# Kaixhin/Rainbow

Measured on AMD Instinct MI355X. Metric: gradient-steps/sec (batch=32, atoms=51), higher is better.
Workload: dtype f32; 1 GPU; pong-canonical-b32; architecture=canonical, batch_per_gpu=32, global_batch=32, atoms=51, actions=6, multi_step=3, replay_capacity_per_gpu=1000000, parallelism=single device

## Files before the change

rainbow_amd/csrc/adam_body.h:

```cpp
#pragma once
#include "rb_common.h"

struct ClipAdamArgs {
  float* p; float* g; float* m; float* v;
  int64_t n;
  const float* part; int nparts;
  float max_norm; float* norm_out;
  float w1, b2, w2, neg_step_size, bc2_sqrt, eps;
  const long long* step_dev;
  double lr, beta1, beta2;
  int64_t skip_lo4, skip_len4;
  const int32_t* batch_status;
  int64_t pair_mu4, pair_len4;
  unsigned hole_lo4, hole4;
  int pair_blk0;
  int pair_f4, pair_split_row;
  float tau;
  const float* pair_eout;
  const float* pair_ein;
  int32_t* pair_clipped;
  float* t;
};
static_assert(sizeof(ClipAdamArgs) <= 256, "ClipAdamArgs: the device copy (adam_args_dev, rb_debug_adam_pass) is 256 bytes");
__device__ __forceinline__ void rb_adam_elem(float& p, float& g, float& m, float& v, float coef, const ClipAdamArgs& a) {
  g = g * coef;
  m = fmaf(a.w1, g - m, m);
  v = v * a.b2 + a.w2 * g * g;
  const float denom = sqrtf(v) / a.bc2_sqrt + a.eps;
  p = p + a.neg_step_size * (m / denom);
}
__device__ __forceinline__ void rb_adam_quad(float4& P, float4& G, float4& M, float4& V, float coef, const ClipAdamArgs& a) {
  rb_adam_elem(P.x, G.x, M.x, V.x, coef, a);
  rb_adam_elem(P.y, G.y, M.y, V.y, coef, a);
  rb_adam_elem(P.z, G.z, M.z, V.z, coef, a);
  rb_adam_elem(P.w, G.w, M.w, V.w, coef, a);
}

__device__ __forceinline__ void rb_ema_elem(float& t, float p, float tau) {
  t = fmaf(tau, p - t, t);
}
__device__ __forceinline__ void rb_ema_quad(float4& T, const float4& P, float tau, bool copy) {
  if (copy) { T = P; return; }
  rb_ema_elem(T.x, P.x, tau); rb_ema_elem(T.y, P.y, tau); rb_ema_elem(T.z, P.z, tau); rb_ema_elem(T.w, P.w, tau);
}

struct rb_adam_req {
  float status;
  unsigned st_lo, st_hi;
  float pv[16];
};
__device__ __forceinline__ void rb_adam_hosted_request(const ClipAdamArgs& a, rb_adam_req& q) {
  const unsigned T = blockDim.x;
  q.status = 0.0f;
  if (a.batch_status) q.status = rb_ld1_buf(rb_make_buf(a.batch_status), 0, 0);
  const rb_buf bs = rb_make_buf(a.step_dev);
  q.st_lo = __builtin_bit_cast(unsigned, rb_ld1_buf(bs, 0, 0)); q.st_hi = __builtin_bit_cast(unsigned, rb_ld1_buf(bs, 4, 0));
  const rb_buf bpart = rb_make_buf(a.part);
#pragma unroll
  for (int u = 0; u < 16; ++u) {
    const int i = (int)threadIdx.x + u * (int)T;
    q.pv[u] = rb_ld1_buf(bpart, 4u * (unsigned)(i < a.nparts ? i : a.nparts - 1), 0);
  }
}
__device__ __forceinline__ bool rb_adam_hosted_prologue(ClipAdamArgs& a, int eb, const rb_adam_req& q, float* s_red16, float* coef_out) {
  const unsigned T = blockDim.x;
  float acc = 0.0f;
#pragma unroll
  for (int u = 0; u < 16; ++u)
    if ((int)threadIdx.x + u * (int)T < a.nparts) acc += q.pv[u];
  {
    const rb_buf bpart = rb_make_buf(a.part);
    for (int i0 = (int)threadIdx.x + 16 * (int)T; i0 < a.nparts; i0 += 16 * (int)T) {
      float pv[16];
#pragma unroll
      for (int u = 0; u < 16; ++u) {
        const int i = i0 + u * (int)T;
        pv[u] = rb_ld1_buf(bpart, 4u * (unsigned)(i < a.nparts ? i : a.nparts - 1), 0);
      }
#pragma unroll
      for (int u = 0; u < 16; ++u)
        if (i0 + u * (int)T < a.nparts) acc += pv[u];
    }
  }
  if (threadIdx.x == 0) {
    const double t = (double)(long long)(((unsigned long long)q.st_hi << 32) | q.st_lo);
    const double bc1 = 1.0 - pow(a.beta1, t), bc2 = 1.0 - pow(a.beta2, t);
    s_red16[16] = (float)(-(a.lr / bc1));
    s_red16[17] = (float)sqrt(bc2);
  }
  acc = rb_block_sum(acc, s_red16);
  if (rb_wave_uniform(__builtin_bit_cast(int, q.status)) != 0) {
    if (eb == 0 && threadIdx.x == 0 && a.norm_out) rb_st1_wt(a.norm_out, 0, 0.0f);
    return false;
  }
  const float total = sqrtf(acc);
  float coef = a.max_norm / (total + 1e-6f);
  if (coef > 1.0f) coef = 1.0f;
  if (eb == 0 && threadIdx.x == 0 && a.norm_out) rb_st1_wt(a.norm_out, 0, total);
  a.neg_step_size = s_red16[16];
  a.bc2_sqrt = s_red16[17];
  *coef_out = coef;
  return true;
}

template <bool EMA>
__device__ __forceinline__ void rb_adam_hosted_pairs(ClipAdamArgs& a, int eb, int pb, float* s_red16) {
  constexpr int PU = 2;
  const unsigned T = blockDim.x;
  const unsigned len4 = (unsigned)a.pair_len4, mu4 = (unsigned)a.pair_mu4;
  const unsigned base = (unsigned)pb * (T * PU) + threadIdx.x;
  rb_adam_req q;
  rb_adam_hosted_request(a, q);
  const rb_buf beo = rb_make_buf(a.pair_eout), bei = rb_make_buf(a.pair_ein);
  float4 E[PU];
  float eo[PU];
#pragma unroll
  for (int u = 0; u < PU; ++u) {
    unsigned j = base + u * T;
    if (j >= len4) j = len4 - 1;
    const unsigned row = j / (unsigned)a.pair_f4, cq = j - row * (unsigned)a.pair_f4;
    eo[u] = rb_ld1_buf(beo, 4 * row, 0);
    E[u] = rb_ld4_buf(bei, 16 * (cq + ((int)row >= a.pair_split_row ? (unsigned)a.pair_f4 : 0u)), 0);
  }
  const rb_buf bp = rb_make_buf(a.p), bg = rb_make_buf(a.g), bm = rb_make_buf(a.m), bv = rb_make_buf(a.v);
  float4 P[PU], G[PU], M[PU], V[PU], P2[PU], M2[PU], V2[PU];
#pragma unroll
  for (int u = 0; u < PU; ++u) {
    unsigned j = base + u * T;
    if (j >= len4) j = len4 - 1;
    const unsigned i = mu4 + j, i2 = i + len4;
    P[u] = rb_ld4_buf(bp, 16 * i, 0); G[u] = rb_ld4_buf(bg, 16 * i, 0);
    M[u] = rb_ld4_buf(bm, 16 * i, 0); V[u] = rb_ld4_buf(bv, 16 * i, 0);
    P2[u] = rb_ld4_buf(bp, 16 * i2, 0); M2[u] = rb_ld4_buf(bm, 16 * i2, 0); V2[u] = rb_ld4_buf(bv, 16 * i2, 0);
  }
  const bool ema_copy = EMA && a.tau == 1.0f;
  float4 TG[EMA ? PU : 1], TG2[EMA ? PU : 1];
  if (EMA && !ema_copy) {
    const rb_buf bt = rb_make_buf(a.t);
#pragma unroll
    for (int u = 0; u < PU; ++u) {
      unsigned j = base + u * T;
      if (j >= len4) j = len4 - 1;
      TG[u] = rb_ld4_buf(bt, 16 * (mu4 + j), 0); TG2[u] = rb_ld4_buf(bt, 16 * (mu4 + j + len4), 0);
    }
  }
  float coef;
  if (!rb_adam_hosted_prologue(a, eb, q, s_red16, &coef)) return;
  if (pb == 0 && threadIdx.x == 0 && a.pair_clipped) rb_st1_wt(reinterpret_cast<float*>(a.pair_clipped), 0, __builtin_bit_cast(float, coef < 1.0f ? 1 : 0));
#pragma unroll
  for (int u = 0; u < PU; ++u) {
    const unsigned j = base + u * T;
    if (j >= len4) continue;
    const unsigned i = mu4 + j, i2 = i + len4;
    float4 pr;
    pr.x = eo[u] * E[u].x; pr.y = eo[u] * E[u].y; pr.z = eo[u] * E[u].z; pr.w = eo[u] * E[u].w;
    float4 G2;
    G2.x = G[u].x * pr.x; G2.y = G[u].y * pr.y; G2.z = G[u].z * pr.z; G2.w = G[u].w * pr.w;
    rb_adam_quad(P[u], G[u], M[u], V[u], coef, a);
    rb_adam_quad(P2[u], G2, M2[u], V2[u], coef, a);
    rb_st4_wt(a.p, 16 * i, P[u]); rb_st4_wt(a.m, 16 * i, M[u]); rb_st4_wt(a.v, 16 * i, V[u]);
    rb_st4_wt(a.p, 16 * i2, P2[u]); rb_st4_wt(a.m, 16 * i2, M2[u]); rb_st4_wt(a.v, 16 * i2, V2[u]);
    if (coef < 1.0f) { rb_st4_wt(a.g, 16 * i, G[u]); rb_st4_wt(a.g, 16 * i2, G2); }
    if (EMA) {
      rb_ema_quad(TG[u], P[u], a.tau, ema_copy); rb_ema_quad(TG2[u], P2[u], a.tau, ema_copy);
      rb_st4_wt(a.t, 16 * i, TG[u]); rb_st4_wt(a.t, 16 * i2, TG2[u]);
    }
  }
}

template <int UNROLL, bool EMA = false>
__device__ __forceinline__ void rb_adam_hosted_block(const ClipAdamArgs* ad, int eb, int nblk, float* s_red16 ) {
  ClipAdamArgs a = rb_ld_uniform(ad);
  const int nplain = a.hole4 > 0 ? a.pair_blk0 : nblk;
  if (eb >= nplain) {
    rb_adam_hosted_pairs<EMA>(a, eb, eb - nplain, s_red16);
    return;
  }
  const unsigned T = blockDim.x;
  const unsigned n4 = (unsigned)(a.n >> 2);
  const unsigned hole_lo = a.hole4 > 0 ? a.hole_lo4 : n4, hole = a.hole4;
  const unsigned nv4 = n4 - hole;
  auto real_of = [&](unsigned j) { return j < hole_lo ? j : j + hole; };
  const unsigned base = (unsigned)eb * (T * UNROLL) + threadIdx.x;
  const rb_buf bp = rb_make_buf(a.p), bg = rb_make_buf(a.g), bm = rb_make_buf(a.m), bv = rb_make_buf(a.v);
  rb_adam_req q;
  rb_adam_hosted_request(a, q);
  float4 P[UNROLL], G[UNROLL], M[UNROLL], V[UNROLL];
#pragma unroll
  for (int u = 0; u < UNROLL; ++u) {
    unsigned j = base + u * T;
    if (j >= nv4) j = nv4 > 0 ? nv4 - 1 : 0;
    const unsigned i = real_of(j);
    P[u] = rb_ld4_buf(bp, 16 * i, 0); G[u] = rb_ld4_buf(bg, 16 * i, 0);
    M[u] = rb_ld4_buf(bm, 16 * i, 0); V[u] = rb_ld4_buf(bv, 16 * i, 0);
  }
  const bool ema_copy = EMA && a.tau == 1.0f;
  const bool has_tail = eb == nplain - 1 && ((a.n >> 2) << 2) + threadIdx.x < a.n;
  const unsigned tail_off = (unsigned)(4 * (((a.n >> 2) << 2) + threadIdx.x));
  float4 TG[EMA ? UNROLL : 1];
  float tg_tail = 0.0f;
  if (EMA && !ema_copy) {
    const rb_buf bt = rb_make_buf(a.t);
#pragma unroll
    for (int u = 0; u < UNROLL; ++u) {
      unsigned j = base + u * T;
      if (j >= nv4) j = nv4 > 0 ? nv4 - 1 : 0;
      TG[u] = rb_ld4_buf(bt, 16 * real_of(j), 0);
    }
    if (has_tail) tg_tail = rb_ld1_buf(bt, tail_off, 0);
  }
  float coef;
  if (!rb_adam_hosted_prologue(a, eb, q, s_red16, &coef)) return;
#pragma unroll
  for (int u = 0; u < UNROLL; ++u) {
    const unsigned j = base + u * T;
    if (j >= nv4) continue;
    const unsigned i = real_of(j);
    rb_adam_quad(P[u], G[u], M[u], V[u], coef, a);
    rb_st4_wt(a.p, 16 * i, P[u]); rb_st4_wt(a.m, 16 * i, M[u]); rb_st4_wt(a.v, 16 * i, V[u]);
    if (coef < 1.0f) rb_st4_wt(a.g, 16 * i, G[u]);
    if (EMA) {
      rb_ema_quad(TG[u], P[u], a.tau, ema_copy);
      rb_st4_wt(a.t, 16 * i, TG[u]);
    }
  }
  if (eb == nplain - 1) {
    const int64_t t = ((a.n >> 2) << 2) + threadIdx.x;
    if (t < a.n) {
      const unsigned o = (unsigned)(4 * t);
      float p = rb_ld1_buf(bp, o, 0), g = rb_ld1_buf(bg, o, 0), m = rb_ld1_buf(bm, o, 0), v = rb_ld1_buf(bv, o, 0);
      rb_adam_elem(p, g, m, v, coef, a);
      rb_st1_wt(a.p, o, p); rb_st1_wt(a.m, o, m); rb_st1_wt(a.v, o, v);
      if (coef < 1.0f) rb_st1_wt(a.g, o, g);
      if (EMA) {
        if (ema_copy) tg_tail = p; else rb_ema_elem(tg_tail, p, a.tau);
        rb_st1_wt(a.t, o, tg_tail);
      }
    }
  }
}

int rb_launch_adam_pending(const ClipAdamArgs* args_dev, int blocks, void* stream, bool ema = false);
```

rainbow_amd/csrc/conv_dispatch.h:

```cpp
#pragma once
#include "learner_plan.h"

static PlanIn plan_in(const rb_learner* l) {
  return PlanIn{l->L, l->opt, l->caps, l->n_cu, l->flags, l->world > 1 && l->fact_local != nullptr && l->caps.fast_fc, l->sink != nullptr};
}

template <class C>
static int launch_conv_fwd(rb_learner* l, int layer, int n_on, int n_tg, const ImgSrc& src, const NetPtrs& on,
                           const NetPtrs& tg, hipStream_t stream) {
  using G = typename C::G;
  constexpr int NT = C::NT, PR = C::PR, KMAX = C::KMAX, PCH = C::PCH;
  constexpr bool FIRST = C::FIRST;
  const ConvLayer& c = l->L.conv[layer];
  const ConvFwdPlan p = plan_conv_fwd_g<C>(plan_in(l), layer, n_on, n_tg, src.f32 != nullptr);
  if (p.kernel == CONV_FWD_GEMM) {
    if (layer == 0) {
      ConvFwdProb<G, true> q;
      q.cin = c.cin; q.cout = c.cout;
      q.n_img[0] = n_on; q.n_img[1] = n_tg; q.img_base[0] = 0; q.img_base[1] = n_on;
      q.w[0] = on.conv_w[0]; q.w[1] = tg.conv_w[0]; q.bias[0] = on.conv_b[0]; q.bias[1] = tg.conv_b[0];
      q.src = src; q.in_f = nullptr; q.out = l->act[0];
      RB_LAUNCH((k_gemm<1, 2, ConvFwdProb<G, true>>), p.grid, dim3(p.block), stream, q);
    } else {
      ConvFwdProb<G, false> q;
      q.cin = c.cin; q.cout = c.cout;
      q.n_img[0] = n_on; q.n_img[1] = n_tg; q.img_base[0] = 0; q.img_base[1] = n_on;
      q.w[0] = on.conv_w[layer]; q.w[1] = tg.conv_w[layer]; q.bias[0] = on.conv_b[layer]; q.bias[1] = tg.conv_b[layer];
      q.src = src; q.in_f = l->act[layer - 1]; q.out = l->act[layer];
      RB_LAUNCH((k_gemm<2, 1, ConvFwdProb<G, false>>), p.grid, dim3(p.block), stream, q);
    }
    RB_LAUNCH_CHECK();
    return RB_OK;
  }
  ConvLdsFwdArgs a;
  a.cin = c.cin; a.cout = c.cout; a.n_on = n_on;
  a.w[0] = on.conv_w[layer]; a.w[1] = tg.conv_w[layer]; a.bias[0] = on.conv_b[layer]; a.bias[1] = tg.conv_b[layer];
  a.src = src; a.in_f = layer > 0 ? l->act[layer - 1] : nullptr; a.out = l->act[layer];
  a.out_blocked = (layer == l->L.nconv - 1 && l->caps.fast_fc) ? l->feat_b : nullptr;
  a.rows_total = n_on + n_tg;
  a.ipb = p.ipb;
  a.img_fast = p.img_fast;
  static const char* const tags[3] = {"conv1_fwd:k_conv_fwd_lds", "conv2_fwd:k_conv_fwd_lds", "conv3_fwd:k_conv_fwd_lds"};
  const dim3 block(p.block);
  switch (p.kernel) {
    case CONV_FWD_FULL:
      if constexpr (FIRST && ConvFwdFullLds<G, KMAX>::FITS) { RB_LAUNCH_T(tags[layer], (k_conv_fwd_full<G, KMAX>), p.grid, block, stream, a); }
      break;
    case CONV_FWD_MULTI_T16:
      if constexpr (!FIRST && C::T16_OK) { RB_LAUNCH_T(tags[layer], (k_conv_fwd_multi_t16<G, NT, PR, KMAX, PCH>), p.grid, block, stream, a); }
      break;
    case CONV_FWD_T16:
      if constexpr (C::T16_OK) { RB_LAUNCH_T(tags[layer], (k_conv_fwd_t16<G, NT, PR, KMAX, FIRST, PCH, 1>), p.grid, block, stream, a); }
      break;
    case CONV_FWD_LDS_F32:
      if constexpr (FIRST) { RB_LAUNCH_T(tags[layer], (k_conv_fwd_lds<G, NT, PR, KMAX, FIRST, PCH, FIRST>), p.grid, block, stream, a); }
      break;
    case CONV_FWD_LDS:
      if constexpr (FIRST || !C::T16_OK) { RB_LAUNCH_T(tags[layer], (k_conv_fwd_lds<G, NT, PR, KMAX, FIRST, PCH>), p.grid, block, stream, a); }
      break;
    case CONV_FWD_GEMM: break;
  }
  RB_LAUNCH_CHECK();
  return RB_OK;
}

static int conv_fwd(rb_learner* l, int layer, int n_on, int n_tg, const ImgSrc& src, const NetPtrs& on,
                    const NetPtrs& tg, hipStream_t stream) {
  return with_geom(l->L.conv[layer], [&](auto cfg) { return launch_conv_fwd<decltype(cfg)>(l, layer, n_on, n_tg, src, on, tg, stream); });
}

template <class C>
static int launch_conv_dx(rb_learner* l, int layer, hipStream_t stream) {
  using G = typename C::G;
  const Layout& L = l->L;
  const ConvLayer& c = L.conv[layer];
  const ConvDxPlan p = plan_conv_dx_g<C>(plan_in(l), layer, l->lazy_dfeat != 0);
  if (p.kernel == CONV_DX_NONE) return RB_OK;
  if constexpr (G::IH != 84) {
    if (p.kernel == CONV_DX_GEMM) {
      ConvDxProb<G> q;
      q.B = L.B; q.cin = c.cin; q.cout = c.cout;
      q.w = l->p_online + L.conv_w[layer]; q.dy = l->dact[layer]; q.x_act = l->act[layer - 1]; q.dx = l->dact[layer - 1];
      if (c.cin <= 32) { RB_LAUNCH((k_gemm<1, 2, ConvDxProb<G>>), p.grid, dim3(p.block), stream, q); }
      else { RB_LAUNCH((k_gemm<2, 1, ConvDxProb<G>>), p.grid, dim3(p.block), stream, q); }
      RB_LAUNCH_CHECK();
      return RB_OK;
    }
    ConvLdsDxArgs a;
    a.cin = c.cin; a.cout = c.cout;
    a.w = l->p_online + L.conv_w[layer]; a.dy = l->dact[layer]; a.x_act = l->act[layer - 1]; a.dx = l->dact[layer - 1];
    a.wT = l->conv_wT[layer];
    constexpr bool lazy = RB_LAST_CONV_GEOM(G);
    a.dy_part = l->dfeat_part; a.dy_mask = l->act[layer]; a.dy_stride = (int64_t)L.B * L.F; a.dy_splits = lazy ? l->lazy_splits : 0;
    a.ipb = p.ipb; a.batch = L.B; a.img_fast = p.img_fast;
    constexpr int NT = ConvDxTiles<G>::NT;
    static const char* const tags[3] = {"conv1_dx:k_conv_dx_lds", "conv2_dx:k_conv_dx_lds", "conv3_dx:k_conv_dx_lds"};
    const dim3 block(p.block);
    switch (p.kernel) {
      case CONV_DX_T16_MULTI:
        if constexpr (dx_t16_geom(G::KS, G::S, G::IH)) { RB_LAUNCH_T(tags[layer], (k_conv_dx_t16_multi<G, 64, lazy>), p.grid, block, stream, a); }
        break;
      case CONV_DX_LDS_MULTI:
        if constexpr (!dx_t16_geom(G::KS, G::S, G::IH)) { RB_LAUNCH_T(tags[layer], (k_conv_dx_lds<G, NT, 64, lazy, true>), p.grid, block, stream, a); }
        break;
      case CONV_DX_LDS:
        RB_LAUNCH_T(tags[layer], (k_conv_dx_lds<G, NT, 64, lazy, false>), p.grid, block, stream, a);
        break;
      default: break;
    }
    RB_LAUNCH_CHECK();
  }
  return RB_OK;
}
static int conv_dx(rb_learner* l, int layer, hipStream_t stream) {
  return with_geom(l->L.conv[layer], [&](auto cfg) { return launch_conv_dx<decltype(cfg)>(l, layer, stream); });
}

template <class C>
static int launch_conv_dw_gemm(rb_learner* l, int layer, const uint8_t* states, hipStream_t stream) {
  using G = typename C::G;
  const Layout& L = l->L;
  const ConvLayer& c = L.conv[layer];
  const ConvDwGemmPlan p = plan_conv_dw_gemm(plan_in(l), layer);
  if (layer == 0) {
    ConvDwProb<G, true> q;
    q.B = L.B; q.cin = c.cin; q.cout = c.cout; q.splits = p.splits;
    q.dy = l->dact[0]; q.x_u8 = states; q.x_f = nullptr; q.part = l->dw_part[0];
    RB_LAUNCH((k_gemm<1, 2, ConvDwProb<G, true>>), p.grid, dim3(p.block), stream, q);
  } else {
    ConvDwProb<G, false> q;
    q.B = L.B; q.cin = c.cin; q.cout = c.cout; q.splits = p.splits;
    q.dy = l->dact[layer]; q.x_u8 = nullptr; q.x_f = l->act[layer - 1]; q.part = l->dw_part[layer];
    RB_LAUNCH((k_gemm<2, 2, ConvDwProb<G, false>>), p.grid, dim3(p.block), stream, q);
  }
  RB_LAUNCH_CHECK();
  l->dw_slices[layer] = p.splits;
  return RB_OK;
}
static int conv_dw_gemm(rb_learner* l, int layer, const uint8_t* states, hipStream_t stream) {
  return with_geom(l->L.conv[layer], [&](auto cfg) { return launch_conv_dw_gemm<decltype(cfg)>(l, layer, states, stream); });
}

static int conv_dw_all(rb_learner* l, hipStream_t stream) {
  const Layout& L = l->L;
  const ConvDwAllPlan p = plan_conv_dw_all(plan_in(l));
  ConvDwAllArgs a;
  a.batch = L.B;
  a.img_fast = p.img_fast;
  for (int i = 0; i < 3; ++i) { a.ipb[i] = p.ipb[i]; a.cotiles[i] = p.cotiles[i]; a.nblocks[i] = p.nblocks[i]; }
  for (int i = 0; i < L.nconv; ++i) {
    const ConvLayer& c = L.conv[i];
    ConvLdsDwArgs& d = a.layer[i];
    d.cin = c.cin; d.cout = c.cout; d.dy = l->dact[i]; d.part = l->dw_part[i];
    d.src = l->cur_src; d.x_f = i > 0 ? l->act[i - 1] : nullptr;
    d.dy_part = l->dfeat_part; d.dy_mask = l->act[i]; d.dy_stride = (int64_t)L.B * L.F;
    d.dy_splits = (l->lazy_dfeat && i == L.nconv - 1 && i > 0) ? l->lazy_splits : 0;
    l->dw_slices[i] = p.dw_slices[i];
  }
  for (int i = L.nconv; i < 3; ++i) a.layer[i] = a.layer[0];
  if (L.nconv == 3) {
    RB_LAUNCH_T("conv_dw_all", (k_conv_dw_all<GeomC1, 7, GeomC2, 9, 512, GeomC3, 7, 576, 3>), dim3(p.total), dim3(RB_CONV_THREADS), stream, a);
  } else {
    RB_LAUNCH_T("conv_dw_all", (k_conv_dw_all<GeomD1, 4, GeomD2, 3, 800, GeomD2, 3, 800, 2>), dim3(p.total), dim3(RB_CONV_THREADS), stream, a);
  }
  RB_LAUNCH_CHECK();
  return RB_OK;
}
```

rainbow_amd/csrc/conv_fwd.h:

```cpp
#pragma once
#include "conv_stage.h"
#include "kernel_stamp.h"

struct ConvLdsFwdArgs {
  int cin, cout;
  int n_on;
  const float* w[2];
  const float* bias[2];
  ImgSrc src;
  const float* in_f;
  float* out;
  float* out_blocked;
  int rows_total;
  int ipb;
  int img_fast;
};

template <class G>
__device__ __forceinline__ void rb_conv_store_out(const ConvLdsFwdArgs& a, int img, int m, int p, float o) {
  a.out[((int64_t)img * a.cout + m) * G::P + p] = o;
  if (a.out_blocked) a.out_blocked[rb_blocked_index(img, m * G::P + p, a.rows_total)] = o;
}

template <class G, int KMAX, int PLANE, int RP, int SUB>
__device__ __forceinline__ constexpr int rb_t16_off(int j) {
  return (j / G::KK) * PLANE + ((j % G::KK) / G::KS) * RP + (((j % G::KK) % G::KS) % G::S) * SUB + ((j % G::KK) % G::KS) / G::S;
}
template <class G, int NT, int PR, int KMAX, int T16 = 0>
struct ConvFwdLdsSize {
  static constexpr int KGRAN = 2 * RB_CONV_WAVES;
  static constexpr int KPAD = (KMAX + KGRAN - 1) / KGRAN * KGRAN;
  static constexpr int RED = RB_CONV_WAVES * 16 * 64;
  static constexpr int WS = KPAD + 4;
  static constexpr int CQ = (KMAX / G::KK) / 4;
  typedef ConvPatch<G, PR, T16 ? CQ : 0> PG;
  static constexpr int SUB = PG::SUB, RP = PG::RP, PLANE = PG::PLANE;
  static __device__ __forceinline__ constexpr int at(int j) { return rb_t16_off<G, KMAX, PLANE, RP, SUB>(j); }
  static constexpr int OPS = 32 * WS + (KMAX / G::KK) * PLANE;
  static constexpr int WSZ = T16 ? OPS : (OPS > RED ? OPS : RED);
  static constexpr int FLOATS = WSZ + (T16 ? 0 : KPAD);
};
template <class G, int NT, int PR, int KMAX, bool FIRST, int PCH = 32 * NT, bool F32SRC = false, int T16 = 0>
struct ConvFwdWaves {
  static constexpr int PT = (PCH + 15) / 16;
  static constexpr bool SPLIT_LAST = T16 == 1 && PT >= 3 && ((2 * PT) % 4) == 2 && ((KMAX / 4) % 8) == 0;
  static constexpr int TILE_WAVES = T16 == 1 ? (SPLIT_LAST ? 2 * PT + 2 : 2 * PT) : PT;
  static constexpr int PARTF = SPLIT_LAST ? 4 * 4 * 64 : 0;
  static constexpr int NWV = T16 == 0 ? RB_CONV_WAVES : (TILE_WAVES + 3) / 4 * 4;
};

struct ConvT16Lane {
  int x, kq, p;
  bool pv;
  const float* bp;
  const float* ap;
};
template <class G, class SZ, int KMAX, int PCH>
__device__ __forceinline__ ConvT16Lane rb_t16_lane(const float* s_w, const float* s_patch, int lane, int p0, int oy0, int pt, int ct0) {
  constexpr int KQ = KMAX / 4, CQ = (KMAX / G::KK) / 4;
  ConvT16Lane L;
  L.x = lane & 15; L.kq = lane >> 4;
  int p = p0 + pt * 16 + L.x;
  L.pv = p < G::P && p < p0 + PCH;
  if (p > G::P - 1) p = G::P - 1;
  L.p = p;
  L.bp = s_patch + L.kq * CQ * SZ::PLANE + (p / G::OH - oy0) * G::S * SZ::RP + (p % G::OH);
  L.ap = s_w + (ct0 * 16 + L.x) * SZ::WS + L.kq * KQ;
  return L;
}
__device__ __forceinline__ void rb_t16_bias(const float* bias, int cout, int m0, float (&b)[4]) {
#pragma unroll
  for (int r = 0; r < 4; ++r) b[r] = bias[m0 + r < cout ? m0 + r : cout - 1];
}

template <class G_, int NT_, int PR_, int KMAX_, bool FIRST_, int PCH_, bool F32SRC, int T16_>
struct ConvFwdCfg {
  typedef G_ G;
  typedef ConvFwdLdsSize<G, NT_, PR_, KMAX_, T16_> SZ;
  typedef typename SZ::PG PG;
  typedef ConvFwdWaves<G, NT_, PR_, KMAX_, FIRST_, PCH_, F32SRC, T16_> WV;
  static constexpr int NT = NT_, PR = PR_, KMAX = KMAX_, PCH = PCH_, T16 = T16_;
  static constexpr bool FIRST = FIRST_;
  static constexpr int NWV = WV::NWV;
  static constexpr int THREADS = 64 * NWV;
  static constexpr int KPAD = SZ::KPAD;
  static constexpr int SUB = SZ::SUB, RP = SZ::RP, PLANE = SZ::PLANE;
  static constexpr int CMAX = KMAX / G::KK;
  static_assert(!T16 || (KMAX % 16 == 0 && CMAX % 4 == 0), "t16: whole float4s per k-slot");
  static constexpr int WS = SZ::WS;
  static constexpr int KW = KPAD / RB_CONV_WAVES;
  static constexpr int HW = KW / 2;
  static constexpr int WR = (32 + NWV - 1) / NWV, WQ = (KMAX + 255) / 256;
  static constexpr bool x_u8 = FIRST && !F32SRC;
  static constexpr bool x_vec = !x_u8 && (G::IH % 4) == 0;
  static constexpr bool x_dw = x_u8 && G::S == 4 && (G::IH % 4) == 0;
  static constexpr int XD = x_dw ? (CMAX * PR * G::IH / 4 + THREADS - 1) / THREADS : 1;
  static constexpr int XU = (x_u8 && !x_dw) ? 2 : 1, XV = x_vec ? 8 : 1, XS = (!x_u8 && !x_vec) ? 12 : 1;
  static constexpr int NF = x_dw ? XD : XU;
  static constexpr int SB = G::KS == 8 ? 0 : G::KS == 4 ? 8 : 16;
  static constexpr int WK = FIRST ? 0 : (G::KS == 3 ? 2 : 1);
};
template <class C>
struct ConvFwdBody {
  typedef typename C::G G;
  typedef typename C::SZ SZ;
  typedef typename C::PG PG;
  static constexpr int THREADS = C::THREADS;
  const ConvLdsFwdArgs& a;
  int t, lane, wave, wgi;
  int img, net, cout0, p0, cin, K, oy0, iy0;
  int rows_valid_w;
  bool w_fast;
  int per_c;
  int v16, total16, v4, total4, total1;
  const float* xbase;
  float* smem;
  float* s_w;
  float* s_patch;
  int* s_koff;
  float4 wv[C::WR][C::WQ];
  int32_t widx[C::NF];
  const uint8_t* fp[C::NF];
  bool fok[C::NF];
  unsigned xd[C::XD];
  uint4 xu[C::XU];
  float4 xv[C::XV];
  float xs[C::XS];

  __device__ __forceinline__ ConvFwdBody(const ConvLdsFwdArgs& a_, int bx, int by, int img_, float* smem_) : a(a_) {
    smem = smem_;
    s_koff = reinterpret_cast<int*>(smem + SZ::WSZ);
    s_w = smem;
    s_patch = smem + 32 * C::WS;
    t = (int)threadIdx.x; lane = t & 63; wave = t >> 6;
    wgi = img_ * 16 + by * 8 + bx;
    img = img_;
    net = img < a.n_on ? 0 : 1;
    cout0 = by * 32;
    p0 = bx * C::PCH;
    cin = a.cin;
    K = cin * G::KK;
    oy0 = p0 / G::OH;
    iy0 = oy0 * G::S;
    int rows = G::IH - iy0;
    if (rows > C::PR) rows = C::PR;
    rows_valid_w = a.cout - cout0 < 32 ? a.cout - cout0 : 32;
    w_fast = (K & 3) == 0 && (K >> 2) <= 64 * C::WQ;
    xbase = C::x_u8 ? nullptr : (C::FIRST ? a.src.f32 + (int64_t)img * cin * G::IP : a.in_f + (int64_t)img * cin * G::IP);
    per_c = rows * G::IH;
    v16 = per_c >> 4; total16 = cin * v16;
    v4 = per_c >> 2; total4 = cin * v4;
    total1 = cin * per_c;
  }

  __device__ __forceinline__ void issue_weights() {
    if (w_fast) {
      const int kq = K >> 2;
#pragma unroll
      for (int r = 0; r < C::WR; ++r) {
        const int m = wave + r * C::NWV;
#pragma unroll
        for (int i = 0; i < C::WQ; ++i) {
          const int q = lane + 64 * i;
          wv[r][i] = make_float4(0.0f, 0.0f, 0.0f, 0.0f);
          if (m < rows_valid_w && q < kq) wv[r][i] = rb_ld4(a.w[net] + (int64_t)(cout0 + m) * K + 4 * q);
        }
      }
    }
  }
// ... 204 lines not shown
    if (wave >= C::WV::TILE_WAVES) return;
    if constexpr (SPLIT_LAST) {
      if (wave >= 2 * PT - 2) {
        t16_half_unit();
        return;
      }
    }
    const int pt = wave % PT, ct0 = (wave / PT) * CTW;
    const ConvT16Lane L = rb_t16_lane<G, SZ, C::KMAX, C::PCH>(s_w, s_patch, lane, p0, oy0, pt, ct0);
    float bias4[CTW][4];
#pragma unroll
    for (int u = 0; u < CTW; ++u) rb_t16_bias(a.bias[net], a.cout, cout0 + (ct0 + u) * 16 + 4 * L.kq, bias4[u]);
    rb_f32x4 acc[CTW];
#pragma unroll
    for (int u = 0; u < CTW; ++u)
#pragma unroll
      for (int r = 0; r < 4; ++r) acc[u][r] = 0.0f;
    rb_t16_steps<SZ, SZ::WS, CTW, 0, KQ / 4>(L.ap, L.bp, acc);
    RB_CSTAMP(C::SB + 2);
    RB_WGT(C::WK, wgi, 4);
#pragma unroll
    for (int u = 0; u < CTW; ++u)
#pragma unroll
      for (int r = 0; r < 4; ++r) {
        const int m = cout0 + (ct0 + u) * 16 + 4 * L.kq + r;
        if (L.pv && m < a.cout) rb_conv_store_out<G>(a, img, m, L.p, fmaxf(acc[u][r] + bias4[u][r], 0.0f));
      }
    RB_CSTAMP(C::SB + 3);
    RB_CSTAMP_LAST(C::SB + 5);
    RB_WGT(C::WK, wgi, 5);
    RB_WGT(C::WK, wgi, 6);
    if constexpr (SPLIT_LAST) __syncthreads();
  }

  __device__ __forceinline__ void mfma_splitk() {
    constexpr int NT = C::NT, KW = C::KW, HW = C::HW, WS = C::WS, RP = C::RP, PCH = C::PCH;
    const int kb = wave * KW;
    int noff[NT];
#pragma unroll
    for (int nt = 0; nt < NT; ++nt) {
      int p = p0 + nt * 32 + (lane & 31);
      if (p > G::P - 1) p = G::P - 1;
      noff[nt] = (p / G::OH - oy0) * G::S * RP + (p % G::OH);
    }
    rb_f32x16 acc[NT];
#pragma unroll
    for (int nt = 0; nt < NT; ++nt)
#pragma unroll
      for (int r = 0; r < 16; ++r) acc[nt][r] = 0.0f;
    const int kh = lane >> 5, ml = lane & 31;
    float bias_r[(16 * 64) / THREADS];
#pragma unroll
    for (int it = 0; it < (16 * 64) / THREADS; ++it) {
      const int idx = t + it * THREADS;
      const int m = cout0 + rb_mfma_row(idx >> 6, idx & 63);
      bias_r[it] = a.bias[net][m < a.cout ? m : a.cout - 1];
    }
    int kos[HW];
#pragma unroll
    for (int j = 0; j < HW; ++j) kos[j] = s_koff[kb + 2 * j + kh];
    const int aswz = (ml >> 3) & 3;
    const int a_even = ml * WS + kb + (kh ^ aswz), a_odd = ml * WS + kb + ((2 + kh) ^ aswz);
#pragma unroll
    for (int j = 0; j < HW; ++j) {
      float av;
      if constexpr (KW % 4 == 0) av = s_w[((j & 1) ? a_odd : a_even) + 4 * (j >> 1)];
      else av = s_w[ml * WS + rb_wswz(ml, kb + 2 * j + kh)];
#pragma unroll
      for (int nt = 0; nt < NT; ++nt) acc[nt] = rb_mfma32(av, s_patch[noff[nt] + kos[j]], acc[nt]);
    }
    RB_CSTAMP(C::SB + 2);
    RB_WGT(C::WK, wgi, 4);
    constexpr int EIT = (16 * 64) / THREADS;
    constexpr bool ONEPASS = NT * SZ::RED <= SZ::WSZ;
    constexpr int TP = ONEPASS ? NT : 1;
#pragma unroll
    for (int nt0 = 0; nt0 < NT; nt0 += TP) {
      __syncthreads();
#pragma unroll
      for (int u = 0; u < TP; ++u)
#pragma unroll
        for (int r = 0; r < 16; ++r) smem[u * SZ::RED + (wave * 16 + r) * 64 + lane] = acc[nt0 + u][r];
      __syncthreads();
#pragma unroll
      for (int u = 0; u < TP; ++u) {
        const int nt = nt0 + u;
#pragma unroll
        for (int it = 0; it < EIT; ++it) {
          const int idx = t + it * THREADS;
          const int l = idx & 63, r = idx >> 6;
          float v = smem[u * SZ::RED + (0 * 16 + r) * 64 + l];
#pragma unroll
          for (int wv_ = 1; wv_ < RB_CONV_WAVES; ++wv_) v += smem[u * SZ::RED + (wv_ * 16 + r) * 64 + l];
          const int m = cout0 + rb_mfma_row(r, l);
          const int p = p0 + nt * 32 + (l & 31);
          if (m < a.cout && p < G::P && p < p0 + PCH)
            rb_conv_store_out<G>(a, img, m, p, fmaxf(v + bias_r[it], 0.0f));
        }
      }
    }
    RB_CSTAMP(C::SB + 3);
    RB_CSTAMP_LAST(C::SB + 5);
    RB_WGT(C::WK, wgi, 5);
    RB_WGT(C::WK, wgi, 6);
  }
};
template <class G, int NT, int PR, int KMAX, bool FIRST, int PCH = 32 * NT, bool F32SRC = false, int T16 = 0>
__device__ __forceinline__ void rb_conv_fwd_body(const ConvLdsFwdArgs& a, int bx, int by, int img, float* smem) {
  typedef ConvFwdCfg<G, NT, PR, KMAX, FIRST, PCH, F32SRC, T16> C;
  ConvFwdBody<C> b(a, bx, by, img, smem);
  RB_CSTAMP(C::SB + 0);
  RB_CSTAMP_LAST(C::SB + 4);
  RB_WGT(C::WK, b.wgi, 0);
  RB_WGT_HW(C::WK, b.wgi);
#if !defined(RB_HOST_INTERP)
  __builtin_amdgcn_s_setprio(3);
#endif
  b.request_window();
  b.issue_weights();
  RB_WGT(C::WK, b.wgi, 1);
  RB_WGT(C::WK, b.wgi, 2);
  b.issue_input();
#if defined(RB_STAMP) && defined(RB_STAMP_FINE)
  RB_WGT(C::WK + 4, b.wgi, 0);
  asm volatile("s_waitcnt vmcnt(0)" ::: "memory");
  RB_WGT(C::WK + 4, b.wgi, 1);
#endif
  b.commit_taps();
  b.commit_weights();
  b.commit_input();
#if defined(RB_STAMP) && defined(RB_STAMP_FINE)
  RB_WGT(C::WK + 4, b.wgi, 2);
#endif
  __syncthreads();
#if !defined(RB_HOST_INTERP)
  __builtin_amdgcn_s_setprio(0);
#endif
  RB_CSTAMP(C::SB + 1);
  RB_WGT(C::WK, b.wgi, 3);
  if constexpr (T16 != 0) b.mfma_t16();
  else b.mfma_splitk();
}

template <class G, int NT, int PR, int KMAX, bool FIRST, int PCH = 32 * NT, bool F32SRC = false>
__global__ __launch_bounds__(RB_CONV_THREADS, (ConvFwdLdsSize<G, NT, PR, KMAX>::FLOATS * 4 <= 80 * 1024 && !F32SRC) ? 4 : 2) void k_conv_fwd_lds(ConvLdsFwdArgs a) {
  __shared__ __attribute__((aligned(16))) float smem[ConvFwdLdsSize<G, NT, PR, KMAX>::FLOATS];
  if (a.img_fast) rb_conv_fwd_body<G, NT, PR, KMAX, FIRST, PCH, F32SRC>(a, (int)blockIdx.z, (int)blockIdx.y, (int)blockIdx.x, smem);
  else rb_conv_fwd_body<G, NT, PR, KMAX, FIRST, PCH, F32SRC>(a, (int)blockIdx.x, (int)blockIdx.y, (int)blockIdx.z, smem);
}

template <class G, int NT, int PR, int KMAX, bool FIRST, int PCH = 32 * NT, int CTW = 1>
__global__ __launch_bounds__((64 * ConvFwdWaves<G, NT, PR, KMAX, FIRST, PCH, false, CTW>::NWV))
void k_conv_fwd_t16(ConvLdsFwdArgs a) {
  __shared__ __attribute__((aligned(16))) float smem[ConvFwdLdsSize<G, NT, PR, KMAX, CTW>::FLOATS + ConvFwdWaves<G, NT, PR, KMAX, FIRST, PCH, false, CTW>::PARTF];
  if (a.img_fast) rb_conv_fwd_body<G, NT, PR, KMAX, FIRST, PCH, false, CTW>(a, (int)blockIdx.z, (int)blockIdx.y, (int)blockIdx.x, smem);
  else rb_conv_fwd_body<G, NT, PR, KMAX, FIRST, PCH, false, CTW>(a, (int)blockIdx.x, (int)blockIdx.y, (int)blockIdx.z, smem);
}

template <class G, int NT, int PR, int KMAX, int PCH = 32 * NT>
__global__ __launch_bounds__((64 * ConvFwdWaves<G, NT, PR, KMAX, false, PCH, false, 1>::NWV))
void k_conv_fwd_multi_t16(ConvLdsFwdArgs a) {
  typedef ConvFwdLdsSize<G, NT, PR, KMAX, 1> SZ;
  typedef ConvFwdWaves<G, NT, PR, KMAX, false, PCH, false, 1> WV;
  constexpr int NWV = WV::NWV, THREADS = 64 * NWV, TILE_WAVES = WV::TILE_WAVES;
  constexpr int WS = SZ::WS, PLANE = SZ::PLANE, CMAX = KMAX / G::KK;
  constexpr int PT = (PCH + 15) / 16, KQ = KMAX / 4;
  static_assert(KMAX % 16 == 0 && CMAX % 4 == 0, "t16: whole float4s per k-slot");
  static_assert(SZ::KPAD == KMAX, "the slab has no padded columns");
  constexpr bool DB = (32 * WS + 2 * CMAX * PLANE) * 4 <= 150 * 1024;
  __shared__ __attribute__((aligned(16))) float smem[SZ::FLOATS + (DB ? CMAX * PLANE : 0)];
  float* s_w = smem;
  float* s_patch = smem + 32 * WS;
  const int t = (int)threadIdx.x, lane = t & 63, wave = t >> 6;
  const int img0 = (a.img_fast ? (int)blockIdx.x : (int)blockIdx.z) * a.ipb;
  const int img_end = img0 + a.ipb < a.rows_total ? img0 + a.ipb : a.rows_total;
  const int cout0 = (int)blockIdx.y * 32;
  const int p0 = (a.img_fast ? (int)blockIdx.z : (int)blockIdx.x) * PCH;
  const int cin = a.cin;
  const int oy0 = p0 / G::OH;
  const int iy0 = oy0 * G::S;
  int rows = G::IH - iy0;
  if (rows > PR) rows = PR;
  const int per_c = rows * G::IH;
  constexpr bool x_vec = (G::IH % 4) == 0;
  constexpr int XV = x_vec ? (CMAX * PR * G::IH / 4 + THREADS - 1) / THREADS : 1;
  constexpr int XS = x_vec ? 1 : (CMAX * PR * G::IH + THREADS - 1) / THREADS;
  const int v4 = per_c >> 2, total4 = cin * v4, total1 = cin * per_c;
  float4 xv[XV];
  float xs[XS];
  auto issue = [&](int img) {
    const float* xbase = a.in_f + (int64_t)img * cin * G::IP;
    if constexpr (x_vec) {
#pragma unroll
      for (int i = 0; i < XV; ++i) {
        const int e = i * THREADS + t;
        const int ec = e < total4 ? e : total4 - 1;
        const int c = ec / v4, q = ec - c * v4;
        xv[i] = rb_ld4(xbase + (int64_t)c * G::IP + iy0 * G::IH + q * 4);
      }
    } else {
#pragma unroll
      for (int i = 0; i < XS; ++i) {
        const int e = i * THREADS + t;
        const int ec = e < total1 ? e : total1 - 1;
        const int c = ec / per_c, q = ec - c * per_c;
        xs[i] = xbase[(int64_t)c * G::IP + iy0 * G::IH + q];
      }
    }
  };
  auto commit = [&](float* dst) {
    if constexpr (x_vec) rb_patch_commit<typename SZ::PG, XV, THREADS>(dst, xv, t, v4, total4);
    else rb_patch_commit<typename SZ::PG, XS, THREADS>(dst, xs, t, per_c, total1);
  };
  const bool tile_wave = wave < TILE_WAVES;
  const int pt = wave % PT, ct0 = (wave / PT) % 2;
  const ConvT16Lane L = rb_t16_lane<G, SZ, KMAX, PCH>(s_w, s_patch, lane, p0, oy0, pt, ct0);
  float bias4[4] = {0.0f, 0.0f, 0.0f, 0.0f};

  auto stage_slab = [&](int img) {
    const int net = img < a.n_on ? 0 : 1;
    rb_slab_copy<KMAX / 4, WS, THREADS>(s_w, a.w[net] + (int64_t)cout0 * KMAX, KMAX, a.cout - cout0 < 32 ? a.cout - cout0 : 32, t);
    rb_t16_bias(a.bias[net], a.cout, cout0 + ct0 * 16 + 4 * L.kq, bias4);
  };
  auto tile = [&](int img, const float* bpi) {
    rb_f32x4 acc[1];
#pragma unroll
    for (int r = 0; r < 4; ++r) acc[0][r] = 0.0f;
    rb_t16_steps<SZ, SZ::WS, 1, 0, KQ / 4>(L.ap, bpi, acc);
#pragma unroll
    for (int r = 0; r < 4; ++r) {
      const int m = cout0 + ct0 * 16 + 4 * L.kq + r;
      if (L.pv && m < a.cout) rb_conv_store_out<G>(a, img, m, L.p, fmaxf(acc[0][r] + bias4[r], 0.0f));
    }
  };

  issue(img0);
  if constexpr (DB) {
    stage_slab(img0);
    commit(s_patch);
    __syncthreads();
    if (img0 + 1 < img_end) issue(img0 + 1);
    int cur = 0;
    for (int img = img0; img < img_end; ++img) {
      if (img != img0 && img == a.n_on) {
        stage_slab(img);
        __syncthreads();
      }
      if (img + 1 < img_end) {
        commit(s_patch + (cur ^ 1) * (CMAX * PLANE));
        if (img + 2 < img_end) issue(img + 2);
      }
      if (tile_wave) tile(img, L.bp + cur * (CMAX * PLANE));
      __syncthreads();
      cur ^= 1;
    }
  } else {
    const int wgt = (int)(blockIdx.x + gridDim.x * (blockIdx.y + gridDim.y * blockIdx.z));
    constexpr int WKM = G::KS == 4 ? 1 : 2;
    (void)wgt; (void)WKM;
    RB_WGT(WKM, wgt, 0);
    for (int img = img0; img < img_end; ++img) {
      if (img == img0 || img == a.n_on) stage_slab(img);
      commit(s_patch);
      __syncthreads();
      if (img == img0) RB_WGT(WKM, wgt, 1);
      if (img == img0 + 1) RB_WGT(WKM, wgt, 3);
      if (img + 1 < img_end) issue(img + 1);
      if (tile_wave) tile(img, L.bp);
      __syncthreads();
      if (img == img0) RB_WGT(WKM, wgt, 2);
      if (img == img0 + 1) RB_WGT(WKM, wgt, 4);
    }
    RB_WGT(WKM, wgt, 5);
    RB_WGT(WKM, wgt, 6);
  }
}

template <class G>
__device__ __forceinline__ constexpr int rb_patch_off(int k) {
  return (k / G::KK) * G::IP + ((k % G::KK) / G::KS) * G::IH + (k % G::KK) % G::KS;
}
template <class G, int KMAX>
struct ConvFwdFullLds {
  static constexpr int KPAD = (KMAX + 1) / 2 * 2;
  static constexpr int CMAX = KMAX / G::KK;
  static constexpr int NTILES = (G::P + 31) / 32;
  static constexpr bool TAIL16 = (G::P % 32) != 0 && (G::P % 32) <= 16 && NTILES == 13 && RB_CONV_WAVES == 8 && (G::KS % 4) == 0 && (CMAX % 2) == 0;
  static constexpr int TAILF = TAIL16 ? 4 * 4 * 64 : 0;
  static constexpr int FLOATS = KPAD * 33 + CMAX * G::IP + TAILF;
  static constexpr bool FITS = FLOATS * 4 <= 160 * 1024 && NTILES <= 2 * RB_CONV_WAVES && (G::IP % 16) == 0;
};
template <class G, int CMAX, int KPAD, int NA>
__device__ __forceinline__ void rb_full_tiles(const float* s_w, const float* s_patch, const int (&noff)[2], int kh, int ml, rb_f32x16 (&acc)[2]) {
  if constexpr (G::KS % 2 == 0) {
    const float* pb0 = s_patch + noff[0] + kh;
    const float* pb1 = s_patch + noff[1] + kh;
    const float* wp = s_w + kh * 33 + ml;
#pragma unroll 1
    for (int c = 0; c < CMAX; ++c) {
#pragma unroll
      for (int jj = 0; jj < G::KK / 2; ++jj) {
        const float av = wp[2 * jj * 33];
        acc[0] = rb_mfma32(av, pb0[rb_patch_off<G>(2 * jj)], acc[0]);
        if constexpr (NA == 2) acc[1] = rb_mfma32(av, pb1[rb_patch_off<G>(2 * jj)], acc[1]);
      }
      pb0 += G::IP; pb1 += G::IP; wp += G::KK * 33;
// ... 143 lines not shown
```

rainbow_amd/csrc/fc_dispatch.h:

```cpp
#pragma once
#include "learner_plan.h"

static NlWeights nl_h(const NetPtrs& p) {
  NlWeights w;
  w.mu = p.h_mu; w.sigma = p.h_sigma; w.eout = p.h_eout; w.ein = p.h_ein; w.bmu = p.h_bmu; w.bsigma = p.h_bsigma;
  return w;
}
static NlWeights nl_z(const NetPtrs& p) {
  NlWeights w;
  w.mu = p.z_mu; w.sigma = p.z_sigma; w.eout = p.z_eout; w.ein = p.z_ein; w.bmu = p.z_bmu; w.bsigma = p.z_bsigma;
  return w;
}

static int fc_forward(rb_learner* l, int n_on, int n_tg, const NetPtrs& on, const NetPtrs& tg, hipStream_t stream) {
  const Layout& L = l->L;
  const int NI = n_on + n_tg;
  const float* feat = l->act[L.nconv - 1];
  const FcFwdPlan p = plan_fc_fwd(plan_in(l), n_on, n_tg);
  if (p.h_kernel == FC_FWD_KGEMM) {
    {
      FcHFwdProb q;
      q.F = L.F; q.H = L.H; q.NI = NI; q.splits = l->caps.hs;
      q.n_img[0] = n_on; q.n_img[1] = n_tg; q.img_base[0] = 0; q.img_base[1] = n_on;
      q.feat = feat; q.net[0] = on; q.net[1] = tg; q.part = l->hpart;
      RB_LAUNCH((k_gemm<2, 2, FcHFwdProb>), p.hgrid, dim3(p.hblock), stream, q);
      RB_LAUNCH_CHECK();
      const int64_t total = (int64_t)NI * 2 * L.H;
      RB_LAUNCH(k_fc_h_finish, dim3((unsigned)rb_div_up(total, 256)), dim3(256), stream, (const float*)l->hpart, l->caps.hs, NI,
                2 * L.H, n_on, on, tg, l->h, (float*)nullptr);
      RB_LAUNCH_CHECK();
    }
    {
      FcZFwdProb q;
      q.H = L.H; q.Z = L.Z; q.NZ = L.NZ;
      q.n_img[0] = n_on; q.n_img[1] = n_tg; q.img_base[0] = 0; q.img_base[1] = n_on;
      q.h = l->h; q.net[0] = on; q.net[1] = tg; q.logits = l->logits;
      RB_LAUNCH((k_gemm<1, 1, FcZFwdProb>), p.zgrid, dim3(p.zblock), stream, q);
      RB_LAUNCH_CHECK();
    }
    return RB_OK;
  }
  if (p.block_copy) {
    RB_LAUNCH(k_block_copy, dim3((unsigned)rb_div_up((int64_t)NI * L.F, 256)), dim3(256), stream, feat, NI, L.F, l->feat_b);
    RB_LAUNCH_CHECK();
  }
  NlFwdArgs a;
  a.x = l->feat_b;
  a.m_base[0] = 0; a.m_cnt[0] = n_on; a.m_base[1] = n_on; a.m_cnt[1] = n_tg;
  a.w[0] = nl_h(on); a.w[1] = nl_h(tg);
  a.K = L.F; a.n_groups = 2;
  const int ht16 = (int)rb_div_up(L.H, 16);
  a.grp[0] = NlRowGroup{0, L.H, 0, 0, 0};
  a.grp[1] = NlRowGroup{L.H, L.H, 0, L.F, ht16};
  a.out = l->h; a.out_blocked = l->h_b; a.ld_out = 2 * L.H; a.rows_total = NI; a.relu = 1;
  switch (p.h_kernel) {
    case FC_FWD_TILED: {
      FcGemmFwdArgs ga;
      ga.f = a;
      ga.mt[0] = p.mt[0]; ga.mt[1] = p.mt[1]; ga.nt = p.nt;
      ga.S = p.S; ga.part = l->gemm_part; ga.ctr = l->gemm_ctr;
      RB_LAUNCH_T("fc_h_fwd:k_fc_gemm_fwd", k_fc_gemm_fwd, p.hgrid, dim3(p.hblock), stream, ga);
      break;
    }
    case FC_FWD_NL3_4: RB_LAUNCH_T("fc_h_fwd:k_nl_fwd3", k_nl_fwd3<4>, p.hgrid, dim3(p.hblock), stream, a); break;
    default: RB_LAUNCH_T("fc_h_fwd:k_nl_fwd3", k_nl_fwd3<2>, p.hgrid, dim3(p.hblock), stream, a); break;
  }
  RB_LAUNCH_CHECK();
  NlFwdArgs z;
  z.x = l->h_b;
  z.m_base[0] = 0; z.m_cnt[0] = n_on; z.m_base[1] = n_on; z.m_cnt[1] = n_tg;
  z.w[0] = nl_z(on); z.w[1] = nl_z(tg);
  z.K = L.H; z.n_groups = 2;
  const int vt16 = (int)rb_div_up(L.Z, 16);
  z.grp[0] = NlRowGroup{0, L.Z, 0, 0, 0};
  z.grp[1] = NlRowGroup{L.Z, L.NZ - L.Z, L.H, L.H, vt16};
  z.out = l->logits; z.out_blocked = nullptr; z.ld_out = L.NZ; z.rows_total = NI; z.relu = 0;
  if (p.z_kernel == FC_FWD_NL3_4) { RB_LAUNCH_T("fc_z_fwd:k_nl_fwd3", k_nl_fwd3<4>, p.zgrid, dim3(p.zblock), stream, z); }
  else { RB_LAUNCH_T("fc_z_fwd:k_nl_fwd3", k_nl_fwd3<2>, p.zgrid, dim3(p.zblock), stream, z); }
  RB_LAUNCH_CHECK();
  return RB_OK;
}

static int forward(rb_learner* l, int n_on, int n_tg, const ImgSrc& src, const NetPtrs& on, const NetPtrs& tg,
                   hipStream_t stream) {
  for (int layer = 0; layer < l->L.nconv; ++layer) {
    int rc = conv_fwd(l, layer, n_on, n_tg, src, on, tg, stream);
    if (rc != RB_OK) return rc;
  }
  return fc_forward(l, n_on, n_tg, on, tg, stream);
}

static NlRowsArgs nl_rows_args(rb_learner* l, const NetPtrs& on, int which, int n, const float* noise_rows) {
  const Layout& L = l->L;
  const NlWeights w = which ? nl_h(on) : nl_z(on);
  const int rows0 = which ? L.H : L.Z;
  NlRowsArgs a;
  a.x = which ? l->feat_b : l->h_b; a.xs = which ? l->feat_s : l->h_s;
  a.mu = w.mu; a.sigma = w.sigma; a.bmu = w.bmu; a.bsigma = w.bsigma;
  a.noise_rows = noise_rows; a.n_noise = (int)L.n_noise; a.eout_off = (int)(which ? L.h_eout : L.z_eout);
  a.M = n; a.K = which ? L.F : L.H; a.n_groups = 2;
  a.grp[0] = NlRowGroup{0, rows0, 0, 0, 0};
  a.grp[1] = NlRowGroup{rows0, which ? L.H : L.NZ - L.Z, which ? 0 : L.H, a.K, (int)rb_div_up(rows0, 16)};
  a.out = which ? l->h : l->logits; a.out_blocked = which ? l->h_b : nullptr; a.out_scaled = which ? l->h_s : nullptr;
  a.next_ein_off = which ? (int)L.z_ein : 0; a.ld_out = which ? 2 * L.H : L.NZ; a.relu = which;
  return a;
}
static NlRowsGenericArgs nl_rows_generic_args(rb_learner* l, const NetPtrs& on, int which, int n, const float* noise_rows) {
  const Layout& L = l->L;
  const NlWeights w = which ? nl_h(on) : nl_z(on);
  NlRowsGenericArgs a;
  a.x = which ? l->act[L.nconv - 1] : l->h; a.ldx = which ? L.F : 2 * L.H;
  a.mu = w.mu; a.sigma = w.sigma; a.bmu = w.bmu; a.bsigma = w.bsigma;
  a.noise_rows = noise_rows; a.n_noise = (int)L.n_noise;
  a.ein_off = (int)(which ? L.h_ein : L.z_ein); a.eout_off = (int)(which ? L.h_eout : L.z_eout);
  a.M = n; a.N = which ? 2 * L.H : L.NZ; a.K = which ? L.F : L.H;
  a.split_row = which ? L.H : L.Z; a.x_off1 = which ? 0 : L.H; a.ein_off1 = a.K;
  a.out = which ? l->h : l->logits; a.ld_out = a.N; a.relu = which;
  return a;
}

static int fc_rows_fwd(rb_learner* l, const ActRowsPlan& p, int n, const float* noise_rows, const NetPtrs& on, hipStream_t stream) {
  const Layout& L = l->L;
  if (p.kernel == ACT_ROWS_GENERIC) {
    const NlRowsGenericArgs h = nl_rows_generic_args(l, on, 1, n, noise_rows), z = nl_rows_generic_args(l, on, 0, n, noise_rows);
    RB_LAUNCH_T("fc_h_rows:k_nlr_generic", k_nlr_generic, p.hgrid, dim3(p.block), stream, h);
    RB_LAUNCH_CHECK();
    RB_LAUNCH_T("fc_z_rows:k_nlr_generic", k_nlr_generic, p.zgrid, dim3(p.block), stream, z);
    RB_LAUNCH_CHECK();
    return RB_OK;
  }
  RB_LAUNCH(k_block_copy_rows, p.copy_grid, dim3(256), stream, (const float*)l->act[L.nconv - 1], n, L.F, noise_rows, (int)L.n_noise,
            (int)L.h_ein, l->feat_b, l->feat_s);
  RB_LAUNCH_CHECK();
  const NlRowsArgs h = nl_rows_args(l, on, 1, n, noise_rows), z = nl_rows_args(l, on, 0, n, noise_rows);
  switch (p.kernel) {
    case ACT_ROWS_NLR_1:
      RB_LAUNCH_T("fc_h_rows:k_nlr_fwd", k_nlr_fwd<1>, p.hgrid, dim3(p.block), stream, h);
      RB_LAUNCH_CHECK();
      RB_LAUNCH_T("fc_z_rows:k_nlr_fwd", k_nlr_fwd<1>, p.zgrid, dim3(p.block), stream, z);
      break;
    default:
      RB_LAUNCH_T("fc_h_rows:k_nlr_fwd", k_nlr_fwd<2>, p.hgrid, dim3(p.block), stream, h);
      RB_LAUNCH_CHECK();
      RB_LAUNCH_T("fc_z_rows:k_nlr_fwd", k_nlr_fwd<2>, p.zgrid, dim3(p.block), stream, z);
      break;
  }
  RB_LAUNCH_CHECK();
  return RB_OK;
}

struct FcDwPlan {
  NlDwArgs a;
  int dw_x, dw_y, slots;
};
static FcDwPlan fc_dw_plan(rb_learner* l, const NetPtrs& on, int which, const float* dy, const float* x, int M, int ct) {
  const Layout& L = l->L;
  FcDwPlan p;
  NlDwArgs& w = p.a;
  memset(&w, 0, sizeof(w));
  w.dy = dy; w.x = x; w.M = M; w.n_prob = 2; w.ct = ct; w.rpb = 0; w.bstride = 0; w.scale = 1.0f; w.sq_part = nullptr;
  w.noise_blocks = nullptr; w.eout_noff = 0; w.ein_noff = 0; w.norm_only = 0; w.no_sigma = 0;
  if (which == 0) {
    const int vt = (int)rb_div_up(L.Z, 16);
    w.ldy = L.NZ; w.ldx = 2 * L.H; w.K = L.H;
    w.prob[0] = NlDwProblem{0, L.Z, 0, 0, 0};
    w.prob[1] = NlDwProblem{L.Z, L.NZ - L.Z, L.H, L.H, vt};
    w.g_mu = l->grads + L.z_mu; w.g_sigma = l->grads + L.z_sigma; w.g_bmu = l->grads + L.z_bmu; w.g_bsigma = l->grads + L.z_bsigma;
    w.eout = on.z_eout; w.ein = on.z_ein;
  } else {
    const int ht = (int)rb_div_up(L.H, 16);
    w.ldy = 2 * L.H; w.ldx = L.F; w.K = L.F;
    w.prob[0] = NlDwProblem{0, L.H, 0, 0, 0};
    w.prob[1] = NlDwProblem{L.H, L.H, 0, L.F, ht};
    w.g_mu = l->grads + L.h_mu; w.g_sigma = l->grads + L.h_sigma; w.g_bmu = l->grads + L.h_bmu; w.g_bsigma = l->grads + L.h_bsigma;
    w.eout = on.h_eout; w.ein = on.h_ein;
  }
  const FcDwTiles t = plan_fc_dw_tiles(L, which, ct);
  p.dw_x = t.dw_x; p.dw_y = t.dw_y; p.slots = t.slots;
  return p;
}

static int fc_backward(rb_learner* l, const NetPtrs& on, float* loss_dev, hipStream_t stream) {
  const Layout& L = l->L;
  const int B = L.B;
  const float* feat = l->act[L.nconv - 1];
  l->exch_pending = 0;
  l->dw_deferred = 0;
  if (!l->caps.fast_fc) {
    const FcBwdPlan p = plan_fc_bwd(plan_in(l), false);
    l->lazy_dfeat = 0;
    l->norm_slots = 0;
    l->sink_done = 0;
    FcGradOut gz;
    gz.g_mu = l->grads + L.z_mu; gz.g_sigma = l->grads + L.z_sigma; gz.g_bmu = l->grads + L.z_bmu;
    gz.g_bsigma = l->grads + L.z_bsigma; gz.eout = on.z_eout; gz.ein = on.z_ein;
    {
      FcZDwProb q;
      q.B = B; q.H = L.H; q.Z = L.Z; q.NZ = L.NZ; q.dlogits = l->dlogits; q.h = l->h; q.o = gz;
      RB_LAUNCH((k_gemm<1, 2, FcZDwProb>), p.gz_dw, dim3(128), stream, q);
      RB_LAUNCH_CHECK();
    }
    {
      FcZDxProb q;
      q.B = B; q.H = L.H; q.Z = L.Z; q.NZ = L.NZ; q.dlogits = l->dlogits; q.h = l->h; q.net = on; q.dh = l->dh;
      RB_LAUNCH((k_gemm<1, 1, FcZDxProb>), p.gz_dx, dim3(64), stream, q);
      RB_LAUNCH_CHECK();
    }
    {
      FcHDwProb q;
      q.B = B; q.H = L.H; q.F = L.F; q.dh = l->dh; q.feat = feat;
      q.o.g_mu = l->grads + L.h_mu; q.o.g_sigma = l->grads + L.h_sigma; q.o.g_bmu = l->grads + L.h_bmu;
      q.o.g_bsigma = l->grads + L.h_bsigma; q.o.eout = on.h_eout; q.o.ein = on.h_ein;
      RB_LAUNCH((k_gemm<2, 2, FcHDwProb>), p.gh_dw, dim3(256), stream, q);
      RB_LAUNCH_CHECK();
    }
    {
      FcHDxProb q;
      q.B = B; q.H = L.H; q.F = L.F; q.splits = l->caps.xs; q.dh = l->dh; q.net = on; q.part = l->dfeat_part;
      RB_LAUNCH((k_gemm<1, 2, FcHDxProb>), p.gh_dx, dim3(128), stream, q);
      RB_LAUNCH_CHECK();
      const int64_t total = (int64_t)B * L.F;
      RB_LAUNCH(k_dfeat_finish, dim3((unsigned)rb_div_up(total, 256)), dim3(256), stream, (const float*)l->dfeat_part,
                l->caps.xs, total, feat, l->dact[L.nconv - 1]);
      RB_LAUNCH_CHECK();
    }
    return RB_OK;
  }
  const PlanIn in = plan_in(l);
  const bool spec = l->spec_now && l->sink && B <= 256 && !in.exch && rb_replay_spec_allowed(l->sink);
  const FcBwdPlan p = plan_fc_bwd(in, spec);
  FcDwPlan zp = fc_dw_plan(l, on, 0, l->dlogits, l->h, B, p.z_ct);
  FcDwPlan hp = fc_dw_plan(l, on, 1, l->dh, feat, B, p.h_ct);
  NlDwArgs& zw = zp.a;
  NlDwArgs& hw_ = hp.a;
  hw_.norm_only = p.defer_dw ? 1 : 0;
  l->dw_deferred = p.defer_dw ? 1 : 0;
  hw_.no_sigma = p.implicit_sigma ? 1 : 0;
  l->sigma_implicit = p.implicit_sigma ? 1 : 0;
  zw.sq_part = p.fuse_norm ? l->norm_part : nullptr;
  hw_.sq_part = p.fuse_norm ? l->norm_part + p.z.slots : nullptr;
  l->norm_slots = p.norm_slots;
// ... 66 lines not shown
```

rainbow_amd/csrc/launch_plan_debug.h:

```cpp
#pragma once
#include "learner_plan.h"

struct PlanText {
  char* out;
  int64_t cap, len;
  bool full;
  void line(const char* fmt, ...) {
    va_list ap;
    va_start(ap, fmt);
    const int64_t room = cap - len;
    const int n = room > 0 ? vsnprintf(out + len, (size_t)room, fmt, ap) : 0;
    va_end(ap);
    if (room <= 0 || n < 0 || n + 1 >= room) { full = true; return; }
    len += n;
    out[len++] = '\n';
    out[len] = 0;
  }
};

static void plan_text_forward(PlanText& t, const PlanIn& in, const char* prefix, int n_on, int n_tg, bool f32) {
  const Layout& L = in.L;
  for (int layer = 0; layer < L.nconv; ++layer) {
    const ConvFwdPlan p = plan_conv_fwd(in, layer, n_on, n_tg, f32);
    char name[96];
    if (p.kernel == CONV_FWD_GEMM) snprintf(name, sizeof(name), "k_gemm<ConvFwdProb<%s>>", p.geom);
    else snprintf(name, sizeof(name), "%s<%s%s>", conv_fwd_kernel_name[p.kernel], p.geom, p.kernel == CONV_FWD_LDS_F32 ? ",F32SRC" : "");
    t.line("%sconv%d_fwd kernel=%s grid=%ux%ux%u block=%u ipb=%d img_fast=%d", prefix, layer + 1, name, p.grid.x, p.grid.y, p.grid.z,
           p.block, p.ipb, p.img_fast);
  }
  const FcFwdPlan f = plan_fc_fwd(in, n_on, n_tg);
  if (f.block_copy) t.line("%sfeat_block_copy kernel=k_block_copy", prefix);
  t.line("%sfc_h_fwd kernel=%s grid=%ux%ux%u block=%u tiles=%d S=%d", prefix, fc_fwd_kernel_name[f.h_kernel], f.hgrid.x, f.hgrid.y,
         f.hgrid.z, f.hblock, f.tiles, f.S);
  if (f.h_kernel == FC_FWD_KGEMM) t.line("%sfc_h_finish kernel=k_fc_h_finish splits=%d", prefix, in.caps.hs);
  t.line("%sfc_z_fwd kernel=%s grid=%ux%ux%u block=%u", prefix, fc_fwd_kernel_name[f.z_kernel], f.zgrid.x, f.zgrid.y, f.zgrid.z, f.zblock);
}

extern "C" int rb_debug_launch_plan(const rb_learner_config_t* cfg, const char* rb_opts, int32_t n_cu, int32_t flags, int32_t world,
                                    int32_t with_sink, char* out, int64_t cap) {
  RB_REQUIRE(out != nullptr && cap >= 1, "rb_debug_launch_plan: no output buffer");
  RB_REQUIRE(n_cu >= 1 && world >= 1, "rb_debug_launch_plan: n_cu and world must be >= 1");
  Layout L;
  int rc = make_layout(cfg, &L);
  if (rc != RB_OK) return rc;
  RbOpts opt;
  rc = rb_opts_parse(rb_opts, &opt);
  if (rc != RB_OK) return rc;
  const LearnerCaps caps = plan_caps(L, opt);
  const PlanIn in{L, opt, caps, n_cu, flags, world > 1 && caps.fast_fc, with_sink != 0};
  PlanText t{out, cap, 0, false};
  out[0] = 0;
  t.line("caps fast_fc=%d fast_conv=%d hs=%d xs=%d ws=%d/%d/%d wT=%d/%d/%d gemm_ws=%d", caps.fast_fc, caps.fast_conv, caps.hs, caps.xs,
         caps.ws[0], caps.ws[1], caps.ws[2], caps.wT[0], caps.wT[1], caps.wT[2], caps.gemm_ws);
  plan_text_forward(t, in, "", 2 * L.B, L.B, false);
  {
    const HeadPlan h = plan_head(in);
    t.line("head kernel=k_head<%d> grid=%ux1x1 block=%d samples=%d tenants=%d waves=%d wt_t16=%d/%d", h.ZI, h.blocks, 64 * h.waves, L.B,
           h.n_jobs > 0 ? 2 * h.per_job : 0, h.waves, h.job_t16[0], h.job_t16[1]);
  }
  const FcBwdPlan b = plan_fc_bwd(in, false);
  if (b.z_kernel == FC_BWD_KGEMM) {
    t.line("fc_z_dw kernel=k_gemm<FcZDwProb> grid=%ux%ux%u block=128", b.gz_dw.x, b.gz_dw.y, b.gz_dw.z);
    t.line("fc_z_dx kernel=k_gemm<FcZDxProb> grid=%ux%ux%u block=64", b.gz_dx.x, b.gz_dx.y, b.gz_dx.z);
    t.line("fc_h_dw kernel=k_gemm<FcHDwProb> grid=%ux%ux%u block=256", b.gh_dw.x, b.gh_dw.y, b.gh_dw.z);
    t.line("fc_h_dx kernel=k_gemm<FcHDxProb> grid=%ux%ux%u block=128", b.gh_dx.x, b.gh_dx.y, b.gh_dx.z);
    t.line("dfeat_finish kernel=k_dfeat_finish splits=%d", b.hsplits);
  } else {
    t.line("fc_z_bwd kernel=%s grid=%ux1x1 block=%u dw=%dx%d dx=%dx%dx%d pipe=%d z_ct=%d z_tall=%d", fc_bwd_kernel_name[b.z_kernel], b.z_blocks,
           b.z_threads, b.zg.dw_x, b.zg.dw_y, b.zg.dx_x, b.zg.dx_y, b.zg.dx_z, b.pipe ? 1 : 0, b.z_ct, b.z_tall ? 1 : 0);
    if (b.pack) t.line("pack_factors kernel=k_pack_factors grid=16x5x1 block=256");
    t.line("fc_h_bwd kernel=%s grid=%ux1x1 block=%u dw=%dx%d dx=%dx%dx%d writeback=%d h_ct=%d gemm_bwd=%d fuse_norm=%d defer_dw=%d "
           "implicit_sigma=%d hsplits=%d rows_per_split=%d norm_slots=%d lazy_dfeat=%d", fc_bwd_kernel_name[b.h_kernel], b.h_blocks, b.h_threads, b.hg.dw_x, b.hg.dw_y,
           b.hg.dx_x, b.hg.dx_y, b.hg.dx_z, b.up_enabled ? 1 : 0, b.h_ct, b.gemm_bwd ? 1 : 0, b.fuse_norm ? 1 : 0, b.defer_dw ? 1 : 0,
           b.implicit_sigma ? 1 : 0, b.hsplits, b.rows_per_split, b.norm_slots, b.lazy_dfeat ? 1 : 0);
    if (!b.lazy_dfeat) t.line("dfeat_finish kernel=k_dfeat_finish splits=%d", b.hsplits);
  }
  auto dx_line = [&](int layer) {
    const ConvDxPlan p = plan_conv_dx(in, layer, b.lazy_dfeat);
    if (p.kernel == CONV_DX_NONE) return;
    char name[96];
    if (p.kernel == CONV_DX_GEMM) snprintf(name, sizeof(name), "k_gemm<ConvDxProb<%s>>", p.geom);
    else if (p.kernel == CONV_DX_T16_MULTI) snprintf(name, sizeof(name), "k_conv_dx_t16_multi<%s>", p.geom);
    else snprintf(name, sizeof(name), "k_conv_dx_lds<%s,MULTI=%s>", p.geom, p.kernel == CONV_DX_LDS_MULTI ? "true" : "false");
    t.line("conv%d_dx kernel=%s grid=%ux%ux%u block=%u ipb=%d img_fast=%d wt_t16=%d", layer + 1, name, p.grid.x, p.grid.y, p.grid.z, p.block,
           p.ipb, p.img_fast, p.wt_t16);
  };
  if (caps.fast_conv) {
    for (int layer = L.nconv - 1; layer > 0; --layer) dx_line(layer);
    const ConvDwAllPlan d = plan_conv_dw_all(in);
    t.line("conv_dw_all kernel=k_conv_dw_all<%d> grid=%ux1x1 block=%d ipb=%d/%d/%d nblocks=%d/%d/%d slices=%d/%d/%d img_fast=%d", L.nconv, d.total,
           RB_CONV_THREADS, d.ipb[0], d.ipb[1], d.ipb[2], d.nblocks[0], d.nblocks[1], d.nblocks[2], d.dw_slices[0], d.dw_slices[1],
           d.dw_slices[2], d.img_fast);
  } else {
    for (int layer = L.nconv - 1; layer >= 0; --layer) {
      const ConvDwGemmPlan d = plan_conv_dw_gemm(in, layer);
      t.line("conv%d_dw kernel=k_gemm<ConvDwProb> grid=%ux%ux%u block=%u splits=%d", layer + 1, d.grid.x, d.grid.y, d.grid.z, d.block, d.splits);
      dx_line(layer);
    }
  }
  t.line("reduce_conv_dw kernel=k_reduce_conv_dw_all grid=%ux1x1 block=64 snapshot=%d", plan_conv_reduce_blocks(L, b.implicit_sigma),
         b.implicit_sigma ? 1 : 0);
  plan_text_forward(t, in, "act_", 1, 0, true);
  {
    int rg[3];
    const bool covered = act_path_covers(L, caps, rg);
    t.line("act_path covered=%d rg=%d/%d/%d", covered ? 1 : 0, rg[0], rg[1], rg[2]);
  }
  if (t.full) {
    rb_set_error("rb_debug_launch_plan: %lld bytes are too few for the plan", (long long)cap);
    return RB_ERR_INVALID;
  }
  return RB_OK;
}
```

rainbow_amd/csrc/learner.hip:

```cpp
#include "learner_internal.h"
#include "kernel_stamp.h"
#include "learner_plan.h"
#include "noise_kernel.h"
#include "grad_finish.h"
#include "head.h"
#include "adam_kernels.h"
#include "noisy_rows.h"
#include "conv_dispatch.h"
#include "fc_dispatch.h"
#include "optimizer_host.h"
#include "param_reset.h"
#include "act_host.h"
#include "exchange_host.h"
#include "layout_api.h"
#include "launch_plan_debug.h"

#if defined(RB_STAMP)
__device__ long long g_span[64];
extern "C" int rb_debug_spans(long long* out, int reset) {
  if (hipMemcpyFromSymbol(out, HIP_SYMBOL(g_span), sizeof(long long) * 64) != hipSuccess) return -2;
  if (reset) {
    long long init[64];
    for (int i = 0; i < 64; ++i) init[i] = (i & 1) ? 0 : 0x7fffffffffffffffLL;
    if (hipMemcpyToSymbol(HIP_SYMBOL(g_span), init, sizeof(init)) != hipSuccess) return -2;
  }
  return 0;
}
__device__ long long g_cstamp[64];
extern "C" int rb_debug_cstamps(long long* out) { return hipMemcpyFromSymbol(out, HIP_SYMBOL(g_cstamp), sizeof(long long) * 64) == hipSuccess ? 0 : -2; }
__device__ long long g_wgt[RB_WGT_KERNELS][RB_WGT_WGS][8];
extern "C" int rb_debug_wgtrace(long long* out, int clear) {
  if (hipMemcpyFromSymbol(out, HIP_SYMBOL(g_wgt), sizeof(long long) * RB_WGT_KERNELS * RB_WGT_WGS * 8) != hipSuccess) return -2;
  if (clear) { void* p = nullptr; if (hipGetSymbolAddress(&p, HIP_SYMBOL(g_wgt)) != hipSuccess || hipMemset(p, 0, sizeof(long long) * RB_WGT_KERNELS * RB_WGT_WGS * 8) != hipSuccess) return -2; }
  return 0;
}
#endif
static void linspace_f32(float start, float end, int steps, float* out) {
  const float step = (end - start) / (float)(steps - 1);
  const int half = steps / 2;
  for (int i = 0; i < steps; ++i)
    out[i] = i < half ? start + step * (float)i : end - step * (float)(steps - i - 1);
}

extern "C" {

int rb_learner_destroy(rb_learner_t* l) {
  if (!l) return RB_OK;
  float** owned[] = {&l->feat_b, &l->h_b, &l->act[0], &l->act[1], &l->act[2], &l->dact[0], &l->dact[1], &l->dact[2], &l->hpart, &l->h,
                     &l->logits, &l->dlogits, &l->dlogitsT, &l->dh, &l->dhT, &l->dfeat_part, &l->dw_part[0], &l->dw_part[1], &l->dw_part[2],
                     &l->conv_wT[0], &l->conv_wT[1], &l->conv_wT[2],
                     &l->log_ps_a, &l->pns_a, &l->m, &l->support, &l->zero_noise, &l->norm_part, &l->gemm_part, &l->noise_snap, &l->feat_s, &l->h_s};
  for (float** p : owned)
    if (*p) rb_dev_free(*p);
  if (l->a_star) rb_dev_free(l->a_star);
  if (l->noise_ctr) rb_dev_free(l->noise_ctr);
  if (l->act_ctr) rb_dev_free(l->act_ctr);
  if (l->gemm_ctr) rb_dev_free(l->gemm_ctr);
  if (l->job_dev) rb_dev_free(l->job_dev);
  if (l->status_copy) rb_dev_free(l->status_copy);
  if (l->adam_args_dev) rb_dev_free(l->adam_args_dev);
  if (l->go_flag) rb_dev_free(l->go_flag);
  delete l;
  return RB_OK;
}

static NoiseMap noise_map(const Layout& L) {
  NoiseMap map;
  const int64_t counts[8] = {L.F, L.H, L.F, L.H, L.H, L.Z, L.H, (int64_t)L.A * L.Z};
  const int64_t dst[8] = {L.h_ein, L.h_eout, L.h_ein + L.F, L.h_eout + L.H, L.z_ein, L.z_eout, L.z_ein + L.H, L.z_eout + L.Z};
  map.seg_begin[0] = 0;
  for (int i = 0; i < 8; ++i) { map.seg_begin[i + 1] = map.seg_begin[i] + (int32_t)counts[i]; map.dst[i] = (int32_t)dst[i]; }
  return map;
}

static NoiseJob make_noise_job(rb_learner* l, int which) {
  NoiseJob j;
  j.noise = which == 1 ? l->n_target : l->n_online;
  j.noise2 = which == 2 ? l->n_target : nullptr;
  j.map = noise_map(l->L);
  j.seed = l->seed; j.ctr = l->noise_ctr;
  j.nblk = (int)rb_div_up(j.map.seg_begin[8], 256); j.nets = which == 2 ? 2 : 1;
  j.dev = l->job_dev + which;
  j.adam_dev = nullptr; j.adam_blocks = 0; j.adam_ema = 0;
  return j;
}
static int upload_noise_jobs(rb_learner* l) {
  if (!l->job_dev) RB_HIP_TRY(rb_dev_malloc((void**)&l->job_dev, 3 * sizeof(NoiseJob)));
  NoiseJob j[3];
  for (int which = 0; which < 3; ++which) j[which] = make_noise_job(l, which);
  RB_HIP_TRY(hipMemcpy(l->job_dev, j, sizeof(j), hipMemcpyHostToDevice));
  return RB_OK;
}

int rb_learner_noise_job(rb_learner_t* l, int32_t which, rb_noise_job_t* out) {
  RB_REQUIRE(l && out, "rb_learner_noise_job: NULL argument");
  RB_REQUIRE(which >= 0 && which <= 2, "rb_learner_noise_job: which must be 0 (online), 1 (target) or 2 (both)");
  static_assert(sizeof(NoiseJob) <= sizeof(rb_noise_job_t), "rb_noise_job_t too small");
  RB_REQUIRE(l->job_dev != nullptr, "rb_learner_noise_job: handle has no device job table");
  const NoiseJob j = make_noise_job(l, which);
  memset(out, 0, sizeof(*out));
  memcpy(out, &j, sizeof(j));
  return RB_OK;
}

int rb_learner_reset_noise(rb_learner_t* l, int32_t which, const float* raw_normals_dev, rb_stream_t stream) {
  RB_REQUIRE(l != nullptr, "rb_learner_reset_noise: NULL handle");
  RB_REQUIRE(which >= 0 && which <= 2, "rb_learner_reset_noise: which must be 0 (online), 1 (target) or 2 (both)");
  RB_REQUIRE(!(which == 2 && raw_normals_dev), "rb_learner_reset_noise: injected normals need one call per net");
  const NoiseMap map = noise_map(l->L);
  float* noise = which == 1 ? l->n_target : l->n_online;
  float* noise2 = which == 2 ? l->n_target : nullptr;
  RB_LAUNCH(k_noise, dim3((unsigned)rb_div_up(map.seg_begin[8], 256), which == 2 ? 2u : 1u), dim3(256), stream, noise, noise2,
            raw_normals_dev, map, l->seed, l->noise_ctr);
  RB_LAUNCH_CHECK();
  return RB_OK;
}

int rb_learner_noise_rows(rb_learner_t* l, int32_t rows, int32_t row0, uint64_t rng_seed, uint64_t rng_round,
                          const float* raw_normals_dev, float* noise_rows_dev, rb_stream_t stream) {
  RB_REQUIRE(l != nullptr, "rb_learner_noise_rows: NULL handle (l)");
  RB_REQUIRE(noise_rows_dev != nullptr, "rb_learner_noise_rows: NULL noise_rows_dev");
  RB_REQUIRE(rows >= 1 && rows <= 256, "rb_learner_noise_rows: rows must be in [1, 256], got %d", (int)rows);
  RB_REQUIRE(row0 >= 0, "rb_learner_noise_rows: row0 must be >= 0, got %d", (int)row0);
  const NoiseMap map = noise_map(l->L);
  const int n_noise = (int)l->L.n_noise;
  RB_LAUNCH(k_noise_rows, dim3((unsigned)rb_div_up(n_noise, 256), (unsigned)rows), dim3(256), stream, noise_rows_dev,
            raw_normals_dev, map, n_noise, rng_seed, rng_round, (int)row0);
  RB_LAUNCH_CHECK();
  return RB_OK;
}

int rb_learner_create(rb_learner_t** out, const rb_learner_config_t* cfg, float* online_params_dev,
                      float* target_params_dev, float* grads_dev, float* online_noise_dev, float* target_noise_dev,
                      uint64_t seed) {
  RB_REQUIRE(out && cfg && online_params_dev && target_params_dev && grads_dev && online_noise_dev && target_noise_dev,
             "rb_learner_create: NULL argument");
  Layout L;
  int rc = make_layout(cfg, &L);
  if (rc != RB_OK) return rc;
  RbOpts opt;
  rc = rb_opts_parse(getenv("RB_OPTS"), &opt);
  if (rc != RB_OK) return rc;
  rb_learner* l = new (std::nothrow) rb_learner();
  if (!l) { rb_set_error("rb_learner_create: host OOM"); return RB_ERR_OOM; }
  memset(l, 0, sizeof(*l));
  l->cfg = *cfg; l->L = L; l->opt = opt;
  l->p_online = online_params_dev; l->p_target = target_params_dev; l->grads = grads_dev;
  l->n_online = online_noise_dev; l->n_target = target_noise_dev;
  l->seed = seed; l->noise_epoch = 0;
  l->world = 1;
  {
    const int64_t seg[6] = {(int64_t)L.B * L.NZ, (int64_t)L.B * 2 * L.H, (int64_t)L.B * 2 * L.H, (int64_t)L.B * L.F, L.n_noise, L.h_mu};
    int64_t off = 0;
    for (int i = 0; i < 6; ++i) { l->fact_off[i] = off; off = align64(off + seg[i]); }
    l->fact_stride = off;
  }
  l->gamma_n = (float)pow(cfg->discount, (double)cfg->multi_step);
  l->delta_z = (float)(((double)cfg->v_max - (double)cfg->v_min) / (double)(cfg->atoms - 1));
  const int B = L.B, NI = 3 * B;
  l->caps = plan_caps(L, l->opt);
#define RB_ALLOC(ptr, count)                                                                         \
  do {                                                                                               \
    hipError_t e_ = rb_dev_malloc((void**)&(ptr), (size_t)(count) * 4);                                  \
    if (e_ != hipSuccess) {                                                                          \
      rb_set_error("rb_learner_create: hipMalloc(%lld B) failed: %s", (long long)(count) * 4, hipGetErrorString(e_)); \
      rb_learner_destroy(l);                                                                         \
      return RB_ERR_OOM;                                                                             \
    }                                                                                                \
  } while (0)
  for (int i = 0; i < L.nconv; ++i) {
    const ConvLayer& c = L.conv[i];
    RB_ALLOC(l->act[i], (int64_t)NI * c.cout * c.P());
    RB_ALLOC(l->dact[i], (int64_t)B * c.cout * c.P());
    {
      int64_t slices = l->caps.ws[i];
      if (slices < (int64_t)B * 5) slices = (int64_t)B * 5;
      RB_ALLOC(l->dw_part[i], slices * c.cout * (c.K() + 1));
    }
    if (l->caps.wT[i]) {
      const int tmax = (c.ks + c.s - 1) / c.s;
      const int64_t n = (int64_t)c.s * c.s * (c.cin / 32) * (rb_div_up(c.cout * tmax * tmax, 16) * 16) * 32;
      RB_ALLOC(l->conv_wT[i], n);
      RB_HIP_TRY(hipMemset(l->conv_wT[i], 0, (size_t)n * 4));
    }
  }
  l->rows_cap = NI;
  RB_ALLOC(l->hpart, (int64_t)l->caps.hs * NI * 2 * L.H);
  RB_ALLOC(l->h, (int64_t)NI * 2 * L.H);
  RB_ALLOC(l->feat_b, (int64_t)NI * (L.F + 16));
  RB_ALLOC(l->h_b, (int64_t)NI * (2 * L.H + 16));
  RB_ALLOC(l->logits, (int64_t)NI * L.NZ);
  RB_ALLOC(l->dlogits, (int64_t)B * L.NZ);
  RB_ALLOC(l->dlogitsT, (int64_t)B * L.NZ);
  RB_ALLOC(l->dh, (int64_t)B * 2 * L.H);
  RB_ALLOC(l->dhT, (int64_t)B * 2 * L.H);
  RB_ALLOC(l->dfeat_part, (int64_t)l->caps.xs * B * L.F);
  RB_ALLOC(l->log_ps_a, (int64_t)B * L.Z);
  RB_ALLOC(l->pns_a, (int64_t)B * L.Z);
  RB_ALLOC(l->m, (int64_t)B * L.Z);
  RB_ALLOC(l->a_star, (int64_t)B);
  RB_ALLOC(l->support, (int64_t)L.Z);
  RB_ALLOC(l->zero_noise, L.n_noise);
  RB_ALLOC(l->noise_snap, L.n_noise);
  RB_ALLOC(l->norm_part, RB_NORM_PART_SLOTS);
  RB_ALLOC(l->noise_ctr, 4);
  RB_ALLOC(l->status_copy, 4);
  RB_ALLOC(l->adam_args_dev, (sizeof(ClipAdamArgs) + 3) / 4);
  RB_ALLOC(l->act_ctr, 6 * RB_FAN_SHARDS * RB_FAN_STRIDE + 32);
#undef RB_ALLOC
  RB_HIP_TRY(hipMemset(l->act_ctr, 0, (6 * RB_FAN_SHARDS * RB_FAN_STRIDE + 32) * 4));
  if (l->opt.spec_draw) {
    hipError_t e = rb_dev_malloc((void**)&l->go_flag, 64);
    if (e != hipSuccess) { rb_set_error("rb_learner_create: hipMalloc failed: %s", hipGetErrorString(e)); rb_learner_destroy(l); return RB_ERR_OOM; }
    RB_HIP_TRY(hipMemset(l->go_flag, 0, 64));
  }
#if defined(RB_HOST_INTERP)
  l->n_cu = 8;
#else
  {
    int dev = 0, cus = 0;
    RB_HIP_TRY(hipGetDevice(&dev));
    RB_HIP_TRY(hipDeviceGetAttribute(&cus, hipDeviceAttributeMultiprocessorCount, dev));
    l->n_cu = cus;
  }
#endif
  if (l->caps.gemm_ws) {
    hipError_t e = rb_dev_malloc((void**)&l->gemm_part, (size_t)l->n_cu * RB_TG_T * RB_TG_T * 4);
    if (e == hipSuccess) e = rb_dev_malloc((void**)&l->gemm_ctr, 1024 * 4);
    if (e != hipSuccess) { rb_set_error("rb_learner_create: hipMalloc failed: %s", hipGetErrorString(e)); rb_learner_destroy(l); return RB_ERR_OOM; }
    RB_HIP_TRY(hipMemset(l->gemm_ctr, 0, 1024 * 4));
  }
  RB_HIP_TRY(hipMemset(l->noise_ctr, 0, 16));
  RB_HIP_TRY(hipMemset(l->status_copy, 0, 16));
  float sup[RB_MAX_ATOMS];
  linspace_f32(cfg->v_min, cfg->v_max, L.Z, sup);
  RB_HIP_TRY(hipMemcpy(l->support, sup, L.Z * sizeof(float), hipMemcpyHostToDevice));
  RB_HIP_TRY(hipMemset(l->zero_noise, 0, L.n_noise * sizeof(float)));
  RB_HIP_TRY(hipMemset(l->hpart, 0, (size_t)l->caps.hs * NI * 2 * L.H * 4));
  {
    const int rc = upload_noise_jobs(l);
    if (rc != RB_OK) return rc;
  }
  *out = l;
  return RB_OK;
}

static int learn_impl(rb_learner_t* l, const ImgSrc& src, const uint8_t* states_dev, const int64_t* actions_dev,
                      const float* returns_dev, const float* nonterminals_dev, const float* weights_dev, float* loss_dev,
                      hipStream_t stream) {
  const Layout& L = l->L;
  const int B = L.B;
  l->cur_src = src;
  const NetPtrs on = net_ptrs(L, l->p_online, l->n_online);
  const NetPtrs tg = net_ptrs(L, l->p_target, l->n_target);
  int rc = forward(l, 2 * B, B, src, on, tg, stream);
  if (rc != RB_OK) return rc;
  {
    const HeadPlan hp = plan_head(plan_in(l));
    HeadTenants tn;
    memset(&tn, 0, sizeof(tn));
    for (int j = 0; j < hp.n_jobs; ++j) {
      const int layer = hp.job_layer[j];
      const ConvLayer& c = L.conv[layer];
      const int tmax = (c.ks + c.s - 1) / c.s;
      tn.job[j] = ConvWtJob{on.conv_w[layer], l->conv_wT[layer], c.cin, c.cout, c.ks, c.s, (int)rb_div_up(c.cout * tmax * tmax, 16) * 16,
                            hp.job_t16[j]};
    }
    if (hp.n_jobs == 1) tn.job[1] = tn.job[0];
    tn.per_job = hp.per_job;
    const dim3 hgrid(hp.blocks), hblock((unsigned)(64 * hp.waves));
#define RB_HEAD_ARGS B, L.Z, L.A, (const float*)l->logits, actions_dev, returns_dev, nonterminals_dev, weights_dev, (const float*)l->support, \
    l->cfg.v_min, l->cfg.v_max, l->gamma_n, l->delta_z, l->log_ps_a, l->pns_a, l->m, l->a_star, loss_dev, l->dlogits, l->step_ctr,          \
    l->batch_status, l->status_copy, l->dlogitsT, tn
    switch (hp.ZI) {
      case 1: RB_LAUNCH_T("head:k_head", k_head<1>, hgrid, hblock, stream, RB_HEAD_ARGS); break;
      case 2: RB_LAUNCH_T("head:k_head", k_head<2>, hgrid, hblock, stream, RB_HEAD_ARGS); break;
      default: RB_LAUNCH_T("head:k_head", k_head<4>, hgrid, hblock, stream, RB_HEAD_ARGS); break;
    }
#undef RB_HEAD_ARGS
  }
  RB_LAUNCH_CHECK();

  const bool exch = plan_in(l).exch;
  if ((rc = fc_backward(l, on, loss_dev, stream)) != RB_OK) return rc;
  if (l->caps.fast_conv) {
    for (int layer = L.nconv - 1; layer > 0; --layer)
      if ((rc = conv_dx(l, layer, stream)) != RB_OK) return rc;
    if ((rc = conv_dw_all(l, stream)) != RB_OK) return rc;
  } else {
    for (int layer = L.nconv - 1; layer >= 0; --layer) {
      if ((rc = conv_dw_gemm(l, layer, states_dev, stream)) != RB_OK) return rc;
      if ((rc = conv_dx(l, layer, stream)) != RB_OK) return rc;
    }
  }
  {
    ReduceAllArgs ra;
    int64_t off = 0;
    for (int layer = 0; layer < L.nconv; ++layer) {
      const ConvLayer& c = L.conv[layer];
      ra.layer[layer] = ReduceLayer{l->dw_part[layer], l->grads + L.conv_w[layer], l->grads + L.conv_b[layer],
                                    l->dw_slices[layer], c.cout, c.K(), off};
      off += (int64_t)c.cout * (c.K() + 1);
    }
    ra.n_layers = L.nconv; ra.total = off;
    ra.sq_part = l->norm_slots > 0 ? l->norm_part + l->norm_conv_base : nullptr;
    ra.grads_base = l->grads;
    ra.copy_base = exch ? l->fact_local + l->fact_off[5] : nullptr;
    ra.snap_src = nullptr; ra.snap_dst = nullptr; ra.snap_n = 0; ra.snap_clear = nullptr;
    if (l->sigma_implicit) { ra.snap_src = l->n_online; ra.snap_dst = l->noise_snap; ra.snap_n = (int)L.n_noise; ra.snap_clear = l->status_copy + 2; }
    RB_LAUNCH(k_reduce_conv_dw_all, dim3(plan_conv_reduce_blocks(L, ra.snap_n > 0)), dim3(64), stream, ra);
    RB_LAUNCH_CHECK();
  }
  return RB_OK;
}

int rb_learner_learn(rb_learner_t* l, const uint8_t* states_dev, const uint8_t* next_states_dev,
                     const int64_t* actions_dev, const float* returns_dev, const float* nonterminals_dev,
                     const float* weights_dev, float* loss_dev, rb_stream_t stream_) {
  RB_REQUIRE(l && states_dev && next_states_dev && actions_dev && returns_dev && nonterminals_dev && weights_dev && loss_dev,
             "rb_learner_learn: NULL argument");
  RB_FLUSH_UPDATE(l, stream_);
  ImgSrc src;
  memset(&src, 0, sizeof(src));
  src.u8_states = states_dev; src.u8_next = next_states_dev; src.B = l->L.B;
  return learn_impl(l, src, states_dev, actions_dev, returns_dev, nonterminals_dev, weights_dev, loss_dev, (hipStream_t)stream_);
}

int rb_learner_learn_windows(rb_learner_t* l, const uint8_t* frames_dev, const int32_t* windows_dev, int32_t window_len,
                             const int64_t* actions_dev, const float* returns_dev, const float* nonterminals_dev,
                             const float* weights_dev, float* loss_dev, rb_stream_t stream_) {
  RB_REQUIRE(l && frames_dev && windows_dev && actions_dev && returns_dev && nonterminals_dev && weights_dev && loss_dev,
             "rb_learner_learn_windows: NULL argument");
  RB_FLUSH_UPDATE(l, stream_);
  RB_REQUIRE(window_len == l->L.hist + l->cfg.multi_step, "rb_learner_learn_windows: window_len must be history + multi_step");
  if (!l->caps.fast_conv) {
    rb_set_error("rb_learner_learn_windows: zero-copy frames need the LDS conv kernels (history <= 4); gather the stacks and "
                 "call rb_learner_learn instead");
    return RB_ERR_STATE;
  }
  ImgSrc src;
  memset(&src, 0, sizeof(src));
  src.B = l->L.B; src.ring = frames_dev; src.win = windows_dev; src.win_len = window_len; src.n_step = l->cfg.multi_step;
  return learn_impl(l, src, nullptr, actions_dev, returns_dev, nonterminals_dev, weights_dev, loss_dev, (hipStream_t)stream_);
}

static int train_step_impl(rb_learner_t* l, const rb_train_step_t* a, rb_comm_t* comm, rb_stream_t stream) {
  RB_REQUIRE(l != nullptr && a != nullptr && a->replay != nullptr, "rb_learner_train_step: NULL argument");
  rb_noise_job_t hosted_job;
  const rb_noise_job_t* job = a->noise_job;
  bool hosted = false;
  if (l->adam_pending) {
    if (job != nullptr && attach_pending_pass(l, job, a->batch, &hosted_job)) {
      job = &hosted_job;
      hosted = true;
    } else {
      const int rc = flush_update(l, (hipStream_t)stream);
      if (rc != RB_OK) return rc;
    }
  }
  {
    auto& t = l->ts_last;
    const bool capturing = l->opt.spec_draw && rb_stream_capturing(stream);
    const bool same = !capturing && t.valid && t.replay == a->replay && t.batch == a->batch && t.max_attempts == a->max_attempts &&
                      t.beta == a->priority_weight &&
                      t.tree_idx == a->tree_idx_dev && t.actions == a->actions_dev && t.returns == a->returns_dev &&
                      t.nonterm == a->nonterminals_dev && t.weights == a->weights_dev && t.mut_after == rb_replay_mutations(a->replay);
    t.streak = same ? t.streak + 1 : 0;
    l->spec_now = (l->opt.spec_draw && t.streak >= 1 && comm == nullptr && a->noise_job != nullptr && a->batch <= 256 && l->caps.fast_fc &&
                   l->sink == a->replay && l->sink_idx == a->tree_idx_dev && rb_replay_spec_allowed(a->replay)) ? 1 : 0;
    if (l->spec_now) {
      rb_spec_request& q = l->spec_req;
      memset(&q, 0, sizeof(q));
      q.batch = a->batch; q.priority_weight = a->priority_weight; q.max_attempts = a->max_attempts;
      q.tree_idx = a->tree_idx_dev; q.actions = a->actions_dev; q.returns = a->returns_dev; q.nonterminals = a->nonterminals_dev;
      q.weights = a->weights_dev;
    }
    if (l->opt.spec_draw && !capturing) rb_replay_spec_arm_accept(a->replay);
  }
  int rc = rb_replay_sample_fused_noise(a->replay, a->batch, a->priority_weight, nullptr, a->max_attempts, a->tree_idx_dev, nullptr,
                                        nullptr, a->actions_dev, a->returns_dev, a->nonterminals_dev, a->weights_dev,
                                        job, stream);
  if (rc != RB_OK) { l->spec_now = 0; return rc; }
  if (hosted) l->adam_pending = 0;
  rc = rb_learner_learn_windows(l, a->frames_dev, rb_replay_current_windows(a->replay), a->window_len, a->actions_dev, a->returns_dev,
                                a->nonterminals_dev, a->weights_dev, a->loss_dev, stream);
  l->spec_now = 0;
  {
    auto& t = l->ts_last;
    t.replay = a->replay; t.batch = a->batch; t.max_attempts = a->max_attempts; t.beta = a->priority_weight; t.tree_idx = a->tree_idx_dev;
    t.actions = a->actions_dev; t.returns = a->returns_dev; t.nonterm = a->nonterminals_dev; t.weights = a->weights_dev;
    t.mut_after = rb_replay_mutations(a->replay); t.valid = rc == RB_OK ? 1 : 0;
  }
  if (rc != RB_OK) return rc;
  if (comm) {
    rc = rb_learner_exchange_rccl(l, comm, stream);
    if (rc != RB_OK) return rc;
  }
  return clip_adam_impl(l, a->max_norm, a->exp_avg_dev, a->exp_avg_sq_dev, a->lr, a->beta1, a->beta2, a->eps, a->step,
                        a->norm_dev, (hipStream_t)stream, (l->flags & RB_LEARNER_DEFER_UPDATE) != 0);
}

int rb_learner_train_step(rb_learner_t* l, const rb_train_step_t* a, rb_stream_t stream) {
  return train_step_impl(l, a, nullptr, stream);
}
int rb_learner_train_step_dist(rb_learner_t* l, const rb_train_step_t* a, rb_comm_t* comm, rb_stream_t stream) {
  RB_REQUIRE(comm != nullptr, "rb_learner_train_step_dist: NULL communicator");
  return train_step_impl(l, a, comm, stream);
}
int rb_learner_set_step_counter(rb_learner_t* l, int64_t* step_dev) {
  RB_REQUIRE(l != nullptr, "rb_learner_set_step_counter: NULL handle");
  l->step_ctr = reinterpret_cast<long long*>(step_dev);
  return RB_OK;
}

int rb_learner_set_flags(rb_learner_t* l, int32_t flags) {
  RB_REQUIRE(l != nullptr, "rb_learner_set_flags: NULL handle");
  RB_REQUIRE((flags & ~(RB_LEARNER_FUSE_FC_H_DW | RB_LEARNER_WRITE_FUSED_GRADS | RB_LEARNER_DEFER_UPDATE | RB_LEARNER_IMPLICIT_SIGMA)) == 0,
             "rb_learner_set_flags: unknown flag bits");
  l->flags = flags;
  return RB_OK;
}

int rb_learner_get_rng(rb_learner_t* l, uint64_t* seed, uint64_t* epoch, rb_stream_t stream) {
  RB_REQUIRE(l && seed && epoch, "rb_learner_get_rng: NULL argument");
  RB_HIP_TRY(hipStreamSynchronize((hipStream_t)stream));
  unsigned long long e = 0;
  RB_HIP_TRY(hipMemcpy(&e, l->noise_ctr, sizeof(e), hipMemcpyDeviceToHost));
  *seed = l->seed; *epoch = (uint64_t)e;
  return RB_OK;
}

int rb_learner_set_rng(rb_learner_t* l, uint64_t seed, uint64_t epoch, rb_stream_t stream) {
  RB_REQUIRE(l != nullptr, "rb_learner_set_rng: NULL handle");
  RB_HIP_TRY(hipStreamSynchronize((hipStream_t)stream));
  const unsigned long long e[2] = {(unsigned long long)epoch, 0ull};
  RB_HIP_TRY(hipMemcpy(l->noise_ctr, e, sizeof(e), hipMemcpyHostToDevice));
  l->seed = seed;
  return upload_noise_jobs(l);
}

int rb_learner_set_priority_sink(rb_learner_t* l, rb_replay_t* replay, const int64_t* tree_idx_dev) {
  RB_REQUIRE(l != nullptr, "rb_learner_set_priority_sink: NULL handle");
  RB_REQUIRE((replay == nullptr) == (tree_idx_dev == nullptr), "rb_learner_set_priority_sink: pass both or neither");
  l->sink = replay;
  l->sink_idx = tree_idx_dev;
  l->batch_status = nullptr;
  if (replay) {
    ReplayView v;
    double omega;
    if (rb_replay_internal_view(replay, &v, &omega) != RB_OK) { rb_set_error("rb_learner_set_priority_sink: bad replay handle"); return RB_ERR_INVALID; }
    l->batch_status = &v.hdr->last_status;
  }
  return RB_OK;
}

int rb_learner_zero_copy_ok(rb_learner_t* l) {
  return (l && l->caps.fast_conv) ? 1 : 0;
}

int rb_learner_priority_written(rb_learner_t* l) {
  return (l && l->sink_done) ? 1 : 0;
}

int rb_learner_grads_modified(rb_learner_t* l) {
  RB_REQUIRE(l != nullptr, "rb_learner_grads_modified: NULL handle");
  if (l->dw_deferred) {
    rb_set_error("rb_learner_grads_modified: the hidden layer's weight gradient was not materialised (RB_LEARNER_FUSE_FC_H_DW)");
    return RB_ERR_STATE;
  }
  if (l->sigma_implicit) {
    rb_set_error("rb_learner_grads_modified: the hidden layer's sigma gradient was not materialised (RB_LEARNER_IMPLICIT_SIGMA): "
                 "call rb_learner_flush before reading or modifying grads_dev");
    return RB_ERR_STATE;
  }
  l->norm_slots = 0;
  return RB_OK;
}

int rb_learner_sync_target(rb_learner_t* l, rb_stream_t stream) {
  RB_REQUIRE(l != nullptr, "rb_learner_sync_target: NULL handle");
  RB_FLUSH_UPDATE(l, stream);
  RB_HIP_TRY(hipMemcpyAsync(l->p_target, l->p_online, (size_t)l->L.n_params * 4, hipMemcpyDeviceToDevice, (hipStream_t)stream));
  RB_HIP_TRY(hipMemcpyAsync(l->n_target, l->n_online, (size_t)l->L.n_noise * 4, hipMemcpyDeviceToDevice, (hipStream_t)stream));
  return RB_OK;
}

#if defined(RB_STAMP)
int rb_debug_occupancy(void) {
  int a = 0, b = 0;
  hipOccupancyMaxActiveBlocksPerMultiprocessor(&a, (const void*)(k_conv_fwd_t16<GeomC1, 3, 20, 256, true, 80, 1>), 640, 0);
  hipOccupancyMaxActiveBlocksPerMultiprocessor(&b, (const void*)(k_conv_fwd_lds<GeomC1, 3, 20, 256, true, 80>), 512, 0);
  hipFuncAttributes fa;
  hipFuncGetAttributes(&fa, (const void*)(k_conv_fwd_t16<GeomC1, 3, 20, 256, true, 80, 1>));
  printf("occupancy API: conv1 t16 (640 threads) %d blocks/CU, conv1 lds (512 threads) %d; t16: regs %d lds %zu maxThreads %d\n", a, b, fa.numRegs, fa.sharedSizeBytes, fa.maxThreadsPerBlock);
  return a;
}
#endif
int rb_learner_debug_read(rb_learner_t* l, int32_t what, void* out_dev, rb_stream_t stream) {
  RB_REQUIRE(l && out_dev, "rb_learner_debug_read: NULL argument");
  if (what < 5) RB_FLUSH_UPDATE(l, stream);
  const Layout& L = l->L;
  const void* src = nullptr;
  size_t bytes = 0;
  switch (what) {
    case 0: src = l->log_ps_a; bytes = (size_t)L.B * L.Z * 4; break;
    case 1: src = l->m; bytes = (size_t)L.B * L.Z * 4; break;
    case 2: src = l->a_star; bytes = (size_t)L.B * 4; break;
    case 3: src = l->pns_a; bytes = (size_t)L.B * L.Z * 4; break;
    case 4: src = l->logits; bytes = (size_t)3 * L.B * L.NZ * 4; break;
    case 5: src = l->h; bytes = (size_t)L.B * 2 * L.H * 4; break;
    case 6: case 7: case 8: {
      const int layer = what - 6;
      RB_REQUIRE(layer < L.nconv, "rb_learner_debug_read: the network has no such conv layer");
      src = l->act[layer]; bytes = (size_t)L.B * L.conv[layer].cout * L.conv[layer].oh * L.conv[layer].oh * 4;
      break;
    }
    default: rb_set_error("rb_learner_debug_read: unknown selector %d", what); return RB_ERR_INVALID;
  }
  RB_HIP_TRY(hipMemcpyAsync(out_dev, src, bytes, hipMemcpyDeviceToDevice, (hipStream_t)stream));
  return RB_OK;
}

}
```

rainbow_amd/csrc/learner_internal.h:

```cpp
#pragma once
#include "conv_fwd.h"
#include "conv_dx.h"
#include "conv_dw.h"
#include "noise_body.h"
#include "adam_body.h"
#include "learner_problems.h"
#include "nl_fwd.h"
#include "nl_bwd.h"
#include "fc_gemm.h"
#include "act_path.h"
#include "rb_common.h"

#include <stdlib.h>

#include <math.h>
#include <string.h>

#include <new>

#define RB_HEAD_MAX_NZ 1408
typedef ConvGeom<8, 4, 84, 20> GeomC1;
typedef ConvGeom<4, 2, 20, 9> GeomC2;
typedef ConvGeom<3, 1, 9, 7> GeomC3;
typedef ConvGeom<5, 5, 84, 16> GeomD1;
typedef ConvGeom<5, 5, 16, 3> GeomD2;
#define RB_LAST_CONV_GEOM(G) (G::KS == 3 || (G::KS == 5 && G::IH == 16))


struct ConvLayer {
  int cin, cout, ks, s, ih, oh;
  int K() const { return cin * ks * ks; }
  int P() const { return oh * oh; }
  int IP() const { return ih * ih; }
};

struct Layout {
  int B, Z, A, H, F, NZ, hist, nconv;
  ConvLayer conv[3];
  int64_t conv_w[3], conv_b[3];
  int64_t h_mu, h_sigma, h_bmu, h_bsigma, z_mu, z_sigma, z_bmu, z_bsigma;
  int64_t n_params;
  int64_t h_ein, h_eout, z_ein, z_eout, n_noise;
};

static int64_t align64(int64_t x) { return (x + 63) / 64 * 64; }

static int make_layout(const rb_learner_config_t* c, Layout* L) {
  RB_REQUIRE(c != nullptr, "learner config is NULL");
  RB_REQUIRE(c->batch >= 1 && c->batch <= 1024, "batch must be in [1,1024]");
  RB_REQUIRE(c->atoms >= 2 && c->atoms <= 256, "atoms must be in [2,256]");
  RB_REQUIRE(c->actions >= 1 && c->actions <= 64, "actions must be in [1,64]");
  RB_REQUIRE(c->atoms * (c->actions + 1) <= RB_HEAD_MAX_NZ, "atoms*(actions+1) must be <= %d (head kernel LDS rows)", RB_HEAD_MAX_NZ);
  RB_REQUIRE(c->history >= 1 && c->history <= 16, "history must be in [1,16]");
  RB_REQUIRE(c->hidden >= 1 && c->hidden <= 8192, "hidden must be in [1,8192]");
  RB_REQUIRE(c->architecture == 0 || c->architecture == 1, "architecture must be 0 (canonical) or 1 (data-efficient)");
  RB_REQUIRE(c->multi_step >= 1, "multi_step must be >= 1");
  RB_REQUIRE(c->v_max > c->v_min, "v_max must exceed v_min");
  memset(L, 0, sizeof(*L));
  L->B = c->batch; L->Z = c->atoms; L->A = c->actions; L->H = c->hidden; L->hist = c->history;
  L->NZ = L->Z + L->A * L->Z;
  if (c->architecture == 0) {
    L->nconv = 3;
    L->conv[0] = ConvLayer{c->history, 32, 8, 4, 84, 20};
    L->conv[1] = ConvLayer{32, 64, 4, 2, 20, 9};
    L->conv[2] = ConvLayer{64, 64, 3, 1, 9, 7};
    L->F = 3136;
  } else {
    L->nconv = 2;
    L->conv[0] = ConvLayer{c->history, 32, 5, 5, 84, 16};
    L->conv[1] = ConvLayer{32, 64, 5, 5, 16, 3};
    L->F = 576;
  }
  int64_t off = 0;
  for (int l = 0; l < L->nconv; ++l) {
    L->conv_w[l] = off; off = align64(off + (int64_t)L->conv[l].cout * L->conv[l].K());
    L->conv_b[l] = off; off = align64(off + L->conv[l].cout);
  }
  const int64_t H2 = 2 * L->H;
  L->h_mu = off; off = align64(off + H2 * L->F);
  L->h_sigma = off; off = align64(off + H2 * L->F);
  L->h_bmu = off; off = align64(off + H2);
  L->h_bsigma = off; off = align64(off + H2);
  L->z_mu = off; off = align64(off + (int64_t)L->NZ * L->H);
  L->z_sigma = off; off = align64(off + (int64_t)L->NZ * L->H);
  L->z_bmu = off; off = align64(off + L->NZ);
  L->z_bsigma = off; off = align64(off + L->NZ);
  L->n_params = off;
  int64_t n = 0;
  L->h_ein = n; n = align64(n + 2 * (int64_t)L->F);
  L->h_eout = n; n = align64(n + H2);
  L->z_ein = n; n = align64(n + H2);
  L->z_eout = n; n = align64(n + L->NZ);
  L->n_noise = n;
  return RB_OK;
}


static NetPtrs net_ptrs(const Layout& L, const float* params, const float* noise) {
  NetPtrs p;
  for (int l = 0; l < 3; ++l) {
    p.conv_w[l] = l < L.nconv ? params + L.conv_w[l] : nullptr;
    p.conv_b[l] = l < L.nconv ? params + L.conv_b[l] : nullptr;
  }
  p.h_mu = params + L.h_mu; p.h_sigma = params + L.h_sigma; p.h_bmu = params + L.h_bmu; p.h_bsigma = params + L.h_bsigma;
  p.z_mu = params + L.z_mu; p.z_sigma = params + L.z_sigma; p.z_bmu = params + L.z_bmu; p.z_bsigma = params + L.z_bsigma;
  p.h_ein = noise + L.h_ein; p.h_eout = noise + L.h_eout; p.z_ein = noise + L.z_ein; p.z_eout = noise + L.z_eout;
  return p;
}

struct RbOpts {
  int generic, fc_gemm, implicit_small, xs, act_fused, spec_draw, spec_stall, img_fast, conv_multi, conv_full, t16, dx_ipb, dw_ipb0, dw_ipb1, dw_ipb2;
};
static const struct { const char* key; int RbOpts::*field; int dflt; const char* what; } rb_opt_table[] = {
  {"generic", &RbOpts::generic, 0, "1: every contraction on the gemm_core.h fallback; 2: the noisy-linear layers only"},
  {"fc_gemm", &RbOpts::fc_gemm, -1, "hidden layer on the LDS-tiled GEMMs of fc_gemm.h: -1 = by shape (from 128 rows per net on), 1 = always, 0 = never"},
  {"implicit_small", &RbOpts::implicit_small, 0, "test hook: RB_LEARNER_IMPLICIT_SIGMA on hidden layers of any size"},
  {"xs", &RbOpts::xs, 0, "row splits of the hidden layer's input gradient: 0 = derived from the hidden size (ceil(2H / 256), at most 4)"},
  {"act_fused", &RbOpts::act_fused, 1, "Agent.act as ONE launch (0: the same kernel, one launch per phase)"},
  {"spec_draw", &RbOpts::spec_draw, 0, "the early draw (opt-in: only append-free loops ever arm it)"},
  {"spec_stall", &RbOpts::spec_stall, 0, "test hook: the early draw's go flag is never stored, the gate in front of the pair expires"},
  {"img_fast", &RbOpts::img_fast, 1, "image-fastest block order of the conv launches (0: the order that image counts off a multiple of 8 get)"},
  {"conv_multi", &RbOpts::conv_multi, -1, "images per workgroup of the conv forward: -1 = by shape (from 256 images on), 0 = one"},
  {"conv_full", &RbOpts::conv_full, 1, "the first layer's whole-image kernel at large batches (0: the chunked kernel)"},
  {"t16", &RbOpts::t16, 1, "the canonical first layer's u8 forward on whole-K 16x16x4 tiles (0: the split-K kernel that history < 4 gets)"},
  {"dx_ipb", &RbOpts::dx_ipb, 0, "images per workgroup of the conv input gradients: 0 = by shape (from batch 64 on)"},
  {"dw_ipb0", &RbOpts::dw_ipb0, 0, "images per workgroup of conv layer 0 in the weight-gradient launch: 0 = by shape"},
  {"dw_ipb1", &RbOpts::dw_ipb1, 0, "... of conv layer 1"},
  {"dw_ipb2", &RbOpts::dw_ipb2, 0, "... of conv layer 2"},
};
static int rb_opts_parse(const char* s, RbOpts* o) {
  for (const auto& row : rb_opt_table) o->*row.field = row.dflt;
  while (s && *s) {
    const char* e = strchr(s, ',');
    const size_t n = e ? (size_t)(e - s) : strlen(s);
    const char* eq = (const char*)memchr(s, '=', n);
    RB_REQUIRE(eq != nullptr && eq > s, "RB_OPTS: entry '%.*s' is not key=value", (int)n, s);
    const size_t kl = (size_t)(eq - s);
    int RbOpts::*field = nullptr;
    for (const auto& row : rb_opt_table)
      if (strlen(row.key) == kl && strncmp(row.key, s, kl) == 0) field = row.field;
    RB_REQUIRE(field != nullptr, "RB_OPTS: unknown key '%.*s'", (int)kl, s);
    char* end = nullptr;
    const long v = strtol(eq + 1, &end, 10);
    RB_REQUIRE(end == s + n && end > eq + 1, "RB_OPTS: key '%.*s' needs an integer value", (int)kl, s);
    o->*field = (int)v;
    s = e ? e + 1 : s + n;
  }
  return RB_OK;
}

struct LearnerCaps {
  int fast_fc;
  int fast_conv;
  int hs, xs, ws[3];
  int wT[3];
  int gemm_ws;
};

struct rb_learner {
  rb_learner_config_t cfg;
  Layout L;
  float *p_online, *p_target, *grads, *n_online, *n_target;
  uint64_t seed;
  uint64_t noise_epoch;
  float* act[3];
  float* dact[3];
  float* hpart;
  float* h;
  float *feat_b, *h_b;
  float *feat_s, *h_s;
  int rows_s_cap;
  float* logits;
  float* dlogits;
  float* dlogitsT;
  float* dh;
  float* dhT;
  float* dfeat_part;
  int lazy_dfeat;
  int lazy_splits;
  RbOpts opt;
  float* gemm_part;
  unsigned* gemm_ctr;
  float* dw_part[3];
  float* conv_wT[3];
  float* log_ps_a;
  float* pns_a;
  float* m;
  int32_t* a_star;
  float* support;
  float* zero_noise;
  float* norm_part;
  int norm_conv_base;
  int norm_slots;
  unsigned long long* noise_ctr;
  NoiseJob* job_dev;
  unsigned* act_ctr;
  unsigned act_epoch;
  int n_cu;
  int rows_cap;
  LearnerCaps caps;
  int dw_slices[3];
  ImgSrc cur_src;
  int sink_done;
  const int32_t* batch_status;
  rb_replay_t* sink;
  const int64_t* sink_idx;
  int world;
  float* fact_local;
  const float* fact_all;
  int64_t fact_off[6];
  int64_t fact_stride;
  int exch_pending;
  long long* step_ctr;
  int flags;
  int dw_deferred;
  ClipAdamArgs* adam_args_dev;
  ClipAdamArgs adam_args_host;
  int adam_args_valid, adam_pending, adam_blocks;
  float target_tau;
  unsigned* go_flag;
  unsigned go_epoch;
  int spec_now;
  rb_spec_request spec_req;
  struct { rb_replay_t* replay; int32_t batch, max_attempts; double beta; int64_t* tree_idx; int64_t* actions; float* returns; float* nonterm;
           float* weights; unsigned long long mut_after; int valid, streak; } ts_last;
  int sigma_implicit;
  float* noise_snap;
  int32_t* status_copy;
  float gamma_n;
  float delta_z;
};

static int flush_update(rb_learner* l, hipStream_t stream);
static int materialize_sigma(rb_learner* l, hipStream_t stream);
int rb_comm_world(const rb_comm_t* comm);
int rb_comm_all_gather_f32(rb_comm_t* comm, const float* send, float* recv, size_t count, hipStream_t stream);

#define RB_FLUSH_UPDATE(l, stream)                                  \
  do {                                                              \
    const int rcf_ = flush_update((l), (hipStream_t)(stream));      \
    if (rcf_ != RB_OK) return rcf_;                                 \
  } while (0)
#define RB_MATERIALIZE_SIGMA(l, stream)                             \
  do {                                                              \
    const int rcm_ = materialize_sigma((l), (hipStream_t)(stream)); \
    if (rcm_ != RB_OK) return rcm_;                                 \
  } while (0)
```

rainbow_amd/csrc/learner_plan.h:

```cpp
#pragma once
#include "learner_internal.h"

#define RB_NORM_PART_SLOTS 16384

struct PlanIn {
  const Layout& L;
  const RbOpts& opt;
  const LearnerCaps& caps;
  int n_cu, flags;
  bool exch;
  bool sink;
};

static int pick_splits(int64_t tiles, int ksteps, int64_t target_blocks) {
  int64_t s = target_blocks / (tiles > 0 ? tiles : 1);
  if (s < 1) s = 1;
  if (s > ksteps) s = ksteps;
  if (s > 64) s = 64;
  const int64_t per = (ksteps + s - 1) / s;
  s = (ksteps + per - 1) / per;
  return (int)s;
}

static LearnerCaps plan_caps(const Layout& L, const RbOpts& opt) {
  LearnerCaps c;
  memset(&c, 0, sizeof(c));
  const int B = L.B;
  const int generic = opt.generic;
  c.fast_fc = (L.F % 32 == 0 && L.H % 32 == 0 && L.F <= RB_NL_FWD_KMAX && L.H <= RB_NL_FWD_KMAX && generic == 0) ? 1 : 0;
  c.fast_conv = (L.hist <= 4 && generic != 1) ? 1 : 0;
  if (c.fast_fc) {
    c.hs = pick_splits(2 * rb_div_up(L.H, 32) * 2 * rb_div_up(2 * B, 64), L.F / 16 / RB_NL_FWD_WAVES, 512);
    c.xs = (int)rb_div_up(2 * L.H, 256);
    if (c.xs > 4) c.xs = 4;
    if (opt.xs > 0) c.xs = opt.xs;
  } else {
    c.hs = pick_splits(rb_div_up(2 * B, 64) * rb_div_up(2 * L.H, 64) * 2, (L.F + 15) / 16, 512);
    c.xs = pick_splits(rb_div_up(B, 32) * rb_div_up(L.F, 64), (2 * L.H + 15) / 16, 512);
  }
  for (int i = 0; i < L.nconv; ++i) {
    const ConvLayer& cl = L.conv[i];
    const int64_t tiles = i == 0 ? rb_div_up(cl.cout, 32) * rb_div_up(cl.K() + 1, 64)
                                 : rb_div_up(cl.cout, 64) * rb_div_up(cl.K() + 1, 64);
    c.ws[i] = pick_splits(tiles, (B * cl.P() + 15) / 16, 512);
    c.wT[i] = (i > 0 && c.fast_conv && cl.cin % 32 == 0) ? 1 : 0;
  }
  c.gemm_ws = (c.fast_fc && opt.fc_gemm != 0) ? 1 : 0;
  return c;
}

template <class G_, int NT_, int PR_, int KMAX_, bool FIRST_, int PCH_ = 32 * NT_>
struct ConvCfg {
  using G = G_;
  static constexpr int NT = NT_, PR = PR_, KMAX = KMAX_, PCH = PCH_;
  static constexpr bool FIRST = FIRST_;
  static constexpr bool T16_OK = KMAX % 16 == 0 && (KMAX / G::KK) % 4 == 0 && 2 * ((PCH + 15) / 16) <= 16 && (PCH % 16 == 0 || PCH >= G::P) && G::P > 16;
};
struct CfgC1 : ConvCfg<GeomC1, 3, 20, 256, true, 80> { static constexpr const char* name = "GeomC1"; };
struct CfgC2 : ConvCfg<GeomC2, 3, 20, 512, false> { static constexpr const char* name = "GeomC2"; };
struct CfgC3 : ConvCfg<GeomC3, 2, 9, 576, false> { static constexpr const char* name = "GeomC3"; };
struct CfgD1 : ConvCfg<GeomD1, 2, 20, 100, true> { static constexpr const char* name = "GeomD1"; };
struct CfgD2 : ConvCfg<GeomD2, 1, 16, 800, false> { static constexpr const char* name = "GeomD2"; };

template <class F>
static auto with_geom(const ConvLayer& c, F&& f) -> decltype(f(CfgC1{})) {
  if (c.ks == 8) return f(CfgC1{});
  if (c.ks == 4) return f(CfgC2{});
  if (c.ks == 3) return f(CfgC3{});
  if (c.ih == 84) return f(CfgD1{});
  return f(CfgD2{});
}

static int round_ipb_to_groups_of_8(int B, int ipb) {
  while (ipb < B && (rb_div_up(B, ipb) % 8 != 0 || B % ipb != 0)) ++ipb;
  return ipb;
}

enum ConvFwdKernel { CONV_FWD_GEMM, CONV_FWD_FULL, CONV_FWD_MULTI_T16, CONV_FWD_T16, CONV_FWD_LDS, CONV_FWD_LDS_F32 };
static const char* const conv_fwd_kernel_name[] = {"k_gemm", "k_conv_fwd_full", "k_conv_fwd_multi_t16", "k_conv_fwd_t16", "k_conv_fwd_lds",
                                                   "k_conv_fwd_lds"};
struct ConvFwdPlan {
  ConvFwdKernel kernel;
  dim3 grid;
  unsigned block;
  int ipb, img_fast;
  const char* geom;
};
template <class C>
static ConvFwdPlan plan_conv_fwd_g(const PlanIn& in, int layer, int n_on, int n_tg, bool f32) {
  using G = typename C::G;
  const ConvLayer& c = in.L.conv[layer];
  const int NI = n_on + n_tg;
  ConvFwdPlan p;
  p.ipb = 1; p.img_fast = 0; p.geom = C::name;
  if (!in.caps.fast_conv) {
    const int n_max = (n_on > n_tg ? n_on : n_tg) * G::P;
    p.kernel = CONV_FWD_GEMM; p.grid = dim3(1, (unsigned)rb_div_up(n_max, layer == 0 ? 64 : 32), 2); p.block = 128;
    return p;
  }
  const bool out_blocked = layer == in.L.nconv - 1 && in.caps.fast_fc;
  const bool multi_forced = in.opt.conv_multi >= 0;
  int ipb = 0;
  if (multi_forced) ipb = in.opt.conv_multi;
  else if (NI >= 256) {
    const int per_img = (int)(rb_div_up(G::P, C::PCH) * rb_div_up(c.cout, 32));
    ipb = (int)rb_div_up((int64_t)NI * per_img, 256);
  }
  if constexpr (C::FIRST && ConvFwdFullLds<G, C::KMAX>::FITS) {
    if (ipb > 0 && !f32 && c.cout <= 32 && !out_blocked && in.opt.conv_full && c.cin * G::KK == C::KMAX && (C::KMAX & 1) == 0) {
      int fi = ipb;
      if (!multi_forced) fi = (int)rb_div_up(NI, 256);
      p.kernel = CONV_FWD_FULL; p.ipb = fi; p.grid = dim3(1, 1, (unsigned)rb_div_up(NI, fi)); p.block = RB_CONV_THREADS;
      return p;
    }
  }
  if constexpr (!C::FIRST && C::T16_OK) {
    if (ipb > 0) {
      const unsigned ngroups = (unsigned)rb_div_up(NI, ipb);
      p.kernel = CONV_FWD_MULTI_T16; p.ipb = ipb;
      p.grid = dim3((unsigned)rb_div_up(G::P, C::PCH), (unsigned)rb_div_up(c.cout, 32), ngroups);
      if (in.opt.img_fast && ngroups % 8 == 0) {
        p.img_fast = 1;
        p.grid = dim3(ngroups, (unsigned)rb_div_up(c.cout, 32), (unsigned)rb_div_up(G::P, C::PCH));
      }
      p.block = 64 * ConvFwdWaves<G, C::NT, C::PR, C::KMAX, false, C::PCH, false, 1>::NWV;
      return p;
    }
  }
  p.grid = dim3((unsigned)rb_div_up(G::P, C::PCH), (unsigned)rb_div_up(c.cout, 32), (unsigned)NI);
  if (in.opt.img_fast && NI % 8 == 0) {
    p.img_fast = 1;
    p.grid = dim3((unsigned)NI, (unsigned)rb_div_up(c.cout, 32), (unsigned)rb_div_up(G::P, C::PCH));
  }
  if constexpr (C::T16_OK) {
    if (!C::FIRST || (in.opt.t16 && !f32 && c.cin * G::KK == C::KMAX)) {
      p.kernel = CONV_FWD_T16; p.block = 64 * ConvFwdWaves<G, C::NT, C::PR, C::KMAX, C::FIRST, C::PCH, false, 1>::NWV;
      return p;
    }
  }
  p.kernel = (C::FIRST && f32) ? CONV_FWD_LDS_F32 : CONV_FWD_LDS; p.block = RB_CONV_THREADS;
  return p;
}
static ConvFwdPlan plan_conv_fwd(const PlanIn& in, int layer, int n_on, int n_tg, bool f32) {
  return with_geom(in.L.conv[layer], [&](auto cfg) { return plan_conv_fwd_g<decltype(cfg)>(in, layer, n_on, n_tg, f32); });
}

static constexpr bool dx_t16_geom(int ks, int s, int ih) { return (ks == 4 && s == 2 && ih == 20) || (ks == 3 && s == 1 && ih == 9); }
static bool dx_uses_t16(const PlanIn& in, int layer) {
  const Layout& L = in.L;
  if (layer < 1 || layer >= L.nconv || !in.caps.fast_conv || !in.caps.wT[layer]) return false;
  const ConvLayer& c = L.conv[layer];
  return dx_t16_geom(c.ks, c.s, c.ih) && (L.B >= 64 || in.opt.dx_ipb > 1);
}
template <class G>
struct ConvDxTiles {
  static constexpr int NPOS = ((G::IH + G::S - 1) / G::S) * ((G::IH + G::S - 1) / G::S);
  static constexpr int NT_ALL = (NPOS + 31) / 32;
  static constexpr int NT = NT_ALL >= 4 ? 2 : 1;
};
enum ConvDxKernel { CONV_DX_NONE, CONV_DX_LDS, CONV_DX_LDS_MULTI, CONV_DX_T16_MULTI, CONV_DX_GEMM };
static const char* const conv_dx_kernel_name[] = {"none", "k_conv_dx_lds", "k_conv_dx_lds", "k_conv_dx_t16_multi", "k_gemm"};
struct ConvDxPlan {
  ConvDxKernel kernel;
  dim3 grid;
  unsigned block;
  int ipb, img_fast;
  int wt_t16;
  const char* geom;
};
template <class C>
static ConvDxPlan plan_conv_dx_g(const PlanIn& in, int layer, bool lazy_dfeat) {
  using G = typename C::G;
  const Layout& L = in.L;
  const ConvLayer& c = L.conv[layer];
  ConvDxPlan p;
  p.kernel = CONV_DX_NONE; p.grid = dim3(0, 0, 0); p.block = 0; p.ipb = 1; p.img_fast = 0; p.geom = C::name;
  p.wt_t16 = dx_uses_t16(in, layer) ? 1 : 0;
  if constexpr (G::IH == 84) {
  } else if (layer > 0 && in.caps.fast_conv && in.caps.wT[layer] && ((lazy_dfeat && layer == L.nconv - 1) == RB_LAST_CONV_GEOM(G))) {
    const unsigned groups = (unsigned)rb_div_up(ConvDxTiles<G>::NT_ALL, ConvDxTiles<G>::NT);
    const int ipb_env = in.opt.dx_ipb;
    const int cit = (int)rb_div_up(c.cin, 32);
    if constexpr (dx_t16_geom(G::KS, G::S, G::IH)) {
      if (p.wt_t16) {
        const int units = G::S * G::S * cit;
        int tp = ipb_env > 0 ? ipb_env : (int)rb_div_up((int64_t)units * L.B, 256);
        if (tp < 1) tp = 1;
        if (ipb_env <= 0 && in.opt.img_fast) tp = round_ipb_to_groups_of_8(L.B, tp);
        const unsigned ng = (unsigned)rb_div_up(L.B, tp);
        p.kernel = CONV_DX_T16_MULTI; p.ipb = tp;
        p.img_fast = (in.opt.img_fast && L.B % tp == 0 && ng % 8 == 0) ? 1 : 0;
        p.grid = p.img_fast ? dim3(ng, (unsigned)cit, (unsigned)(G::S * G::S)) : dim3((unsigned)(G::S * G::S), (unsigned)cit, ng);
        p.block = 64 * ConvDxT16<G, 64>::NWV;
        return p;
      }
    }
    const int per_img = (G::S * G::S) * (int)groups * cit;
    int ipb = 1;
    if (ipb_env > 0) ipb = ipb_env;
    else if (L.B >= 64) {
      while (per_img * (int)rb_div_up(L.B, ipb) > 256) ++ipb;
      if (in.opt.img_fast) ipb = round_ipb_to_groups_of_8(L.B, ipb);
    }
    p.ipb = ipb;
    p.grid = dim3((unsigned)(G::S * G::S) * groups, (unsigned)cit, (unsigned)rb_div_up(L.B, ipb));
    if (in.opt.img_fast && L.B % ipb == 0 && (L.B / ipb) % 8 == 0) {
      p.img_fast = 1;
      p.grid = dim3((unsigned)(L.B / ipb), (unsigned)cit, (unsigned)(G::S * G::S) * groups);
    }
    p.kernel = (!dx_t16_geom(G::KS, G::S, G::IH) && ipb > 1) ? CONV_DX_LDS_MULTI : CONV_DX_LDS;
    p.block = RB_CONV_THREADS;
  } else if (layer > 0) {
    const int nyy = (G::IH + G::S - 1) / G::S;
    const int n_max = L.B * nyy * nyy;
    p.kernel = CONV_DX_GEMM; p.block = 128;
    p.grid = c.cin <= 32 ? dim3(1, (unsigned)rb_div_up(n_max, 64), (unsigned)(G::S * G::S))
                         : dim3((unsigned)rb_div_up(c.cin, 64), (unsigned)rb_div_up(n_max, 32), (unsigned)(G::S * G::S));
  }
  return p;
}
static ConvDxPlan plan_conv_dx(const PlanIn& in, int layer, bool lazy_dfeat) {
  return with_geom(in.L.conv[layer], [&](auto cfg) { return plan_conv_dx_g<decltype(cfg)>(in, layer, lazy_dfeat); });
}

struct ConvDwAllPlan {
  int ipb[3], cotiles[3], nblocks[3], dw_slices[3];
  int img_fast;
  unsigned total;
};
static ConvDwAllPlan plan_conv_dw_all(const PlanIn& in) {
  const Layout& L = in.L;
  ConvDwAllPlan p;
  memset(&p, 0, sizeof(p));
  const int ipb_all = L.B > 32 ? (int)rb_div_up(L.B, 32) : 1;
  bool uniform = true;
  for (int i = 0; i < 3; ++i) p.ipb[i] = ipb_all;
  if (L.B > 32 && L.nconv == 3) {
    const int cost[3] = {75, 74, 62};
    const int chunks0 = (L.conv[0].oh + 6) / 7, ct[3] = {(int)rb_div_up(L.conv[0].cout, 32), (int)rb_div_up(L.conv[1].cout, 32), (int)rb_div_up(L.conv[2].cout, 32)};
    int best_t = ipb_all * cost[0], best[3] = {ipb_all, ipb_all, ipb_all};
    for (int i0 = 1; i0 <= ipb_all; ++i0)
      for (int i1 = 1; i1 <= ipb_all + 4; ++i1)
        for (int i2 = 1; i2 <= ipb_all + 4; ++i2) {
          const int wgs = chunks0 * ct[0] * (int)rb_div_up(L.B, i0) + ct[1] * (int)rb_div_up(L.B, i1) + ct[2] * (int)rb_div_up(L.B, i2);
          if (wgs > in.n_cu) continue;
          int t = i0 * cost[0];
          if (i1 * cost[1] > t) t = i1 * cost[1];
          if (i2 * cost[2] > t) t = i2 * cost[2];
          if (t < best_t) { best_t = t; best[0] = i0; best[1] = i1; best[2] = i2; }
        }
    for (int i = 0; i < 3; ++i) p.ipb[i] = best[i];
  }
  const int dw_ipb[3] = {in.opt.dw_ipb0, in.opt.dw_ipb1, in.opt.dw_ipb2};
  for (int i = 0; i < L.nconv; ++i) {
    if (dw_ipb[i] > 0) p.ipb[i] = dw_ipb[i];
    if (p.ipb[i] > L.B) p.ipb[i] = L.B;
    if (p.ipb[i] != ipb_all) uniform = false;
    const int groups = (int)rb_div_up(L.B, p.ipb[i]);
    const ConvLayer& c = L.conv[i];
    const int rc = i == 0 ? (c.ks == 8 ? 7 : 4) : c.oh;
    const int chunks = (c.oh + rc - 1) / rc;
    p.cotiles[i] = (int)rb_div_up(c.cout, 32);
    p.nblocks[i] = chunks * p.cotiles[i] * groups;
    p.dw_slices[i] = chunks * groups;
    p.total += (unsigned)p.nblocks[i];
  }
  for (int i = L.nconv; i < 3; ++i) { p.nblocks[i] = 0; p.cotiles[i] = 1; }
  p.img_fast = (in.opt.img_fast && uniform && (int)rb_div_up(L.B, ipb_all) % 8 == 0 && p.nblocks[0] % 8 == 0 && p.nblocks[1] % 8 == 0) ? 1 : 0;
  return p;
}
struct ConvDwGemmPlan { dim3 grid; unsigned block; int splits; };
static ConvDwGemmPlan plan_conv_dw_gemm(const PlanIn& in, int layer) {
  const ConvLayer& c = in.L.conv[layer];
  ConvDwGemmPlan p;
  p.splits = in.caps.ws[layer];
  p.grid = dim3((unsigned)rb_div_up(c.cout, layer == 0 ? 32 : 64), (unsigned)rb_div_up(c.K() + 1, 64), (unsigned)p.splits);
  p.block = layer == 0 ? 128 : 256;
  return p;
}

static bool fc_uses_gemm(const PlanIn& in, int rows) {
  return in.caps.gemm_ws && (in.opt.fc_gemm == 1 || (in.opt.fc_gemm < 0 && rows >= 128));
}
enum FcFwdKernel { FC_FWD_KGEMM, FC_FWD_NL3_2, FC_FWD_NL3_4, FC_FWD_TILED };
static const char* const fc_fwd_kernel_name[] = {"k_gemm", "k_nl_fwd3<2>", "k_nl_fwd3<4>", "k_fc_gemm_fwd"};
struct FcFwdPlan {
  FcFwdKernel h_kernel, z_kernel;
  dim3 hgrid, zgrid;
  unsigned hblock, zblock;
  int block_copy;
  int mt[2], nt, tiles, S;
};
static FcFwdPlan plan_fc_fwd(const PlanIn& in, int n_on, int n_tg) {
  const Layout& L = in.L;
  FcFwdPlan p;
  memset(&p, 0, sizeof(p));
  const int m_max = n_on > n_tg ? n_on : n_tg;
// ... 191 lines not shown
```

rainbow_amd/csrc/optimizer_host.h:

```cpp
#pragma once
#include "learner_plan.h"

static int materialize_sigma(rb_learner* l, hipStream_t stream) {
  if (!l->sigma_implicit) return RB_OK;
  const Layout& L = l->L;
  const NetPtrs sn = net_ptrs(L, l->p_online, l->noise_snap);
  const int64_t len4 = (int64_t)2 * L.H * L.F / 4;
  RB_LAUNCH(k_materialize_sigma, dim3((unsigned)rb_div_up(len4, 256 * 4)), dim3(256), stream, l->grads, L.h_mu / 4, len4, L.F / 4, L.H,
            sn.h_eout, sn.h_ein, (const int32_t*)(l->status_copy + 2));
  RB_LAUNCH_CHECK();
  l->sigma_implicit = 0;
  return RB_OK;
}

static int flush_update(rb_learner* l, hipStream_t stream) {
  if (!l->adam_pending) return RB_OK;
  FusedDwAdamArgs f;
  memset(&f, 0, sizeof(f));
  ClipAdamArgs a = l->adam_args_host;
  int blocks = l->adam_blocks;
  if (a.pair_len4 > 0) {
    const int rc = rb_launch_adam_pending(l->adam_args_dev, blocks, stream, a.t != nullptr);
    if (rc != RB_OK) return rc;
    l->adam_pending = 0;
    return RB_OK;
  }
  if (a.t) RB_LAUNCH_T("clip_adam:k_clip_adam", (k_clip_adam<4, true, false, true>), dim3((unsigned)blocks), dim3(256), stream, a, f);
  else RB_LAUNCH_T("clip_adam:k_clip_adam", (k_clip_adam<4, true, false>), dim3((unsigned)blocks), dim3(256), stream, a, f);
  RB_LAUNCH_CHECK();
  l->adam_pending = 0;
  return RB_OK;
}

static int sumsq_pass(rb_learner* l, hipStream_t stream, int* nparts) {
  const int64_t n = l->L.n_params;
  *nparts = plan_sumsq_blocks(n);
  RB_LAUNCH(k_sumsq, dim3((unsigned)*nparts), dim3(256), stream, (const float*)l->grads, n, l->norm_part);
  RB_LAUNCH_CHECK();
  return RB_OK;
}

static bool attach_pending_pass(rb_learner* l, const rb_noise_job_t* job_in, int32_t batch, rb_noise_job_t* job_out) {
  memcpy(job_out, job_in, sizeof(*job_out));
  if (!l->adam_pending || batch > 256) return false;
  NoiseJob* nj = reinterpret_cast<NoiseJob*>(job_out);
  nj->adam_dev = l->adam_args_dev; nj->adam_blocks = l->adam_blocks;
  nj->adam_ema = l->adam_args_host.t != nullptr ? 1 : 0;
  return true;
}

static int launch_target_ema(rb_learner* l, float tau, const int32_t* status, hipStream_t stream) {
  const int64_t n = l->L.n_params;
  const int64_t n4 = n >> 2;
  RB_LAUNCH_T("clip_adam:k_target_ema", k_target_ema, dim3((unsigned)rb_div_up(n4 > 0 ? n4 : 1, 256 * 4)), dim3(256), stream, l->p_target,
              (const float*)l->p_online, n, tau, status);
  RB_LAUNCH_CHECK();
  return RB_OK;
}

static int clip_adam_impl(rb_learner* l, float max_norm, float* exp_avg, float* exp_avg_sq, double lr, double beta1, double beta2,
                          double eps, int64_t step, float* norm_dev, hipStream_t stream, bool defer) {
  RB_REQUIRE(exp_avg != nullptr && exp_avg_sq != nullptr, "rb_learner_clip_adam: NULL moment buffer");
  RB_REQUIRE(step >= 1 || (step == 0 && l->step_ctr), "rb_learner_clip_adam: step is 1-based (0 = take it from the device counter set "
             "with rb_learner_set_step_counter)");
  const int64_t n = l->L.n_params;
  int nparts = l->norm_slots;
  if (!(max_norm < INFINITY) && norm_dev == nullptr) {
    nparts = 0;
  } else if (nparts <= 0) {
    const int rcs = sumsq_pass(l, stream, &nparts);
    if (rcs != RB_OK) return rcs;
  }
  l->norm_slots = 0;
  ClipAdamArgs a;
  memset(&a, 0, sizeof(a));
  a.p = l->p_online; a.g = l->grads; a.m = exp_avg; a.v = exp_avg_sq; a.n = n;
  a.part = l->norm_part; a.nparts = nparts; a.max_norm = max_norm; a.norm_out = norm_dev;
  const double bc1 = 1.0 - pow(beta1, (double)step), bc2 = 1.0 - pow(beta2, (double)step);
  a.w1 = (float)(1.0 - beta1); a.b2 = (float)beta2; a.w2 = (float)(1.0 - beta2);
  a.neg_step_size = (float)(-(lr / bc1)); a.bc2_sqrt = (float)sqrt(bc2); a.eps = (float)eps;
  a.step_dev = step == 0 ? l->step_ctr : nullptr; a.lr = lr; a.beta1 = beta1; a.beta2 = beta2;
  a.batch_status = l->status_copy;
  const bool ema = l->target_tau > 0.0f;
  if (ema && !l->dw_deferred) { a.t = l->p_target; a.tau = l->target_tau; }
  const int64_t n4 = n >> 2;
  RB_REQUIRE(n * 4 < (int64_t)0x7fffffff, "rb_learner_clip_adam: the flat parameter buffer must be smaller than 2 GiB");
  FusedDwAdamArgs f;
  memset(&f, 0, sizeof(f));
  a.skip_lo4 = 0; a.skip_len4 = 0;
  if (l->dw_deferred) {
    const Layout& L = l->L;
    const NetPtrs on = net_ptrs(L, l->p_online, l->n_online);
    FcDwPlan hp = fc_dw_plan(l, on, 1, l->dh, l->act[L.nconv - 1], L.B, 0);
    f.dw = hp.a;
    f.mu_off = L.h_mu; f.sigma_off = L.h_sigma;
    f.dw_x = hp.dw_x; f.n_tile_blocks = 2 * hp.dw_x * hp.dw_y;
    f.write_grads = (l->flags & RB_LEARNER_WRITE_FUSED_GRADS) ? 1 : 0;
    a.skip_lo4 = L.h_mu >> 2; a.skip_len4 = (L.h_bmu - L.h_mu) >> 2;
    const unsigned grid = (unsigned)(f.n_tile_blocks + rb_div_up(n4 - a.skip_len4 > 0 ? n4 - a.skip_len4 : 1, 256 * 4));
    RB_LAUNCH_T("clip_adam:k_clip_adam", (k_clip_adam<4, true, true>), dim3(grid), dim3(256), stream, a, f);
    l->dw_deferred = 0;
    if (ema) {
      RB_LAUNCH_CHECK();
      return launch_target_ema(l, l->target_tau, a.batch_status, stream);
    }
  } else {
    unsigned grid = (unsigned)rb_div_up(n4 > 0 ? n4 : 1, 256 * 4);
    const bool will_defer = defer && a.step_dev != nullptr && a.nparts > 0 && l->adam_args_dev != nullptr;
    if (l->sigma_implicit && will_defer) {
      const Layout& L = l->L;
      const NetPtrs sn = net_ptrs(L, l->p_online, l->noise_snap);
      a.pair_mu4 = L.h_mu / 4; a.pair_len4 = (int64_t)2 * L.H * L.F / 4;
      a.pair_f4 = L.F / 4; a.pair_split_row = L.H; a.pair_eout = sn.h_eout; a.pair_ein = sn.h_ein;
      a.pair_clipped = l->status_copy + 2;
      a.hole_lo4 = (unsigned)a.pair_mu4; a.hole4 = (unsigned)(2 * a.pair_len4);
      a.pair_blk0 = (int)rb_div_up(n4 - 2 * a.pair_len4 > 0 ? n4 - 2 * a.pair_len4 : 1, 256 * 4);
      grid = (unsigned)(a.pair_blk0 + rb_div_up(a.pair_len4, 256 * 2));
    } else if (l->sigma_implicit) {
      const int rcm = materialize_sigma(l, stream);
      if (rcm != RB_OK) return rcm;
    }
    if (will_defer) {
      if (!l->adam_args_valid || memcmp(&a, &l->adam_args_host, sizeof(a)) != 0) {
        RB_LAUNCH(k_store_adam_args, dim3(1), dim3(64), stream, a, l->adam_args_dev);
        RB_LAUNCH_CHECK();
        memcpy(&l->adam_args_host, &a, sizeof(a));
        l->adam_args_valid = 1;
      }
      l->adam_pending = 1;
      l->adam_blocks = (int)grid;
      return RB_OK;
    }
    if (ema) RB_LAUNCH_T("clip_adam:k_clip_adam", (k_clip_adam<4, true, false, true>), dim3(grid), dim3(256), stream, a, f);
    else RB_LAUNCH_T("clip_adam:k_clip_adam", (k_clip_adam<4, true, false>), dim3(grid), dim3(256), stream, a, f);
  }
  RB_LAUNCH_CHECK();
  return RB_OK;
}

extern "C" {

int rb_learner_set_target_tau(rb_learner_t* l, float tau, rb_stream_t stream) {
  RB_REQUIRE(l != nullptr, "rb_learner_set_target_tau: NULL handle");
  RB_REQUIRE(tau >= 0.0f && tau <= 1.0f, "rb_learner_set_target_tau: tau must be in [0, 1], got %g", (double)tau);
  RB_FLUSH_UPDATE(l, stream);
  l->target_tau = tau;
  return RB_OK;
}

int rb_learner_target_ema(rb_learner_t* l, float tau, rb_stream_t stream) {
  RB_REQUIRE(l != nullptr, "rb_learner_target_ema: NULL handle");
  RB_REQUIRE(tau >= 0.0f && tau <= 1.0f, "rb_learner_target_ema: tau must be in [0, 1], got %g", (double)tau);
  RB_FLUSH_UPDATE(l, stream);
  if (tau == 0.0f) return RB_OK;
  return launch_target_ema(l, tau, nullptr, (hipStream_t)stream);
}

int rb_learner_flush(rb_learner_t* l, rb_stream_t stream) {
  RB_REQUIRE(l != nullptr, "rb_learner_flush: NULL handle");
  const int rc = flush_update(l, (hipStream_t)stream);
  if (rc != RB_OK) return rc;
  return materialize_sigma(l, (hipStream_t)stream);
}

int rb_learner_attach_pending(rb_learner_t* l, const rb_noise_job_t* job_in, int32_t batch, rb_noise_job_t* job_out) {
  if (!l || !job_in || !job_out) { rb_set_error("rb_learner_attach_pending: NULL argument"); return RB_ERR_INVALID; }
  return attach_pending_pass(l, job_in, batch, job_out) ? 1 : 0;
}
int rb_learner_pending_launched(rb_learner_t* l) {
  RB_REQUIRE(l != nullptr, "rb_learner_pending_launched: NULL handle");
  l->adam_pending = 0;
  return RB_OK;
}
static int debug_adam_pass_impl(int32_t form, float* p, float* g, float* m, float* v, int64_t n, const float* part, int32_t nparts,
                               float max_norm, float* norm_out, const long long* step_dev, int64_t step, double lr, double beta1,
                               double beta2, double eps, const int32_t* batch_status, int64_t pair_mu4, int64_t pair_len4, int32_t pair_f4,
                               int32_t pair_split_row, const float* pair_eout, const float* pair_ein, int32_t* pair_clipped, void* args_dev,
                               float* target, float tau, rb_stream_t stream_) {
  hipStream_t stream = (hipStream_t)stream_;
  RB_REQUIRE(p && g && m && v && part && n >= 0 && n * 4 < (int64_t)0x7fffffff && nparts > 0, "rb_debug_adam_pass: bad buffers");
  RB_REQUIRE(form == 0 ? (step >= 1 && pair_len4 == 0) : (form == 1 && step_dev && args_dev), "rb_debug_adam_pass: bad form");
  static_assert(sizeof(ClipAdamArgs) <= 256, "rb_debug_adam_pass: args_dev is documented as 256 bytes");
  ClipAdamArgs a;
  memset(&a, 0, sizeof(a));
  a.p = p; a.g = g; a.m = m; a.v = v; a.n = n;
  a.part = part; a.nparts = nparts; a.max_norm = max_norm; a.norm_out = norm_out;
  const double bc1 = 1.0 - pow(beta1, (double)step), bc2 = 1.0 - pow(beta2, (double)step);
  a.w1 = (float)(1.0 - beta1); a.b2 = (float)beta2; a.w2 = (float)(1.0 - beta2);
  a.neg_step_size = (float)(-(lr / bc1)); a.bc2_sqrt = (float)sqrt(bc2); a.eps = (float)eps;
  a.step_dev = form == 1 ? step_dev : nullptr; a.lr = lr; a.beta1 = beta1; a.beta2 = beta2;
  a.batch_status = batch_status;
  a.t = target; a.tau = target ? tau : 0.0f;
  const int64_t n4 = n >> 2;
  unsigned grid = (unsigned)rb_div_up(n4 > 0 ? n4 : 1, 256 * 4);
  if (form == 0) {
    FusedDwAdamArgs f;
    memset(&f, 0, sizeof(f));
    if (target) RB_LAUNCH((k_clip_adam<4, true, false, true>), dim3(grid), dim3(256), stream, a, f);
    else RB_LAUNCH((k_clip_adam<4, true, false>), dim3(grid), dim3(256), stream, a, f);
    RB_LAUNCH_CHECK();
    return RB_OK;
  }
  if (pair_len4 > 0) {
    RB_REQUIRE(pair_mu4 >= 0 && pair_mu4 + 2 * pair_len4 <= n4 && pair_f4 > 0 && pair_len4 % pair_f4 == 0 && pair_eout && pair_ein,
               "rb_debug_adam_pass: bad pair range");
    a.pair_mu4 = pair_mu4; a.pair_len4 = pair_len4; a.pair_f4 = pair_f4; a.pair_split_row = pair_split_row;
    a.pair_eout = pair_eout; a.pair_ein = pair_ein; a.pair_clipped = pair_clipped;
    a.hole_lo4 = (unsigned)pair_mu4; a.hole4 = (unsigned)(2 * pair_len4);
    a.pair_blk0 = (int)rb_div_up(n4 - 2 * pair_len4 > 0 ? n4 - 2 * pair_len4 : 1, 256 * 4);
    grid = (unsigned)(a.pair_blk0 + rb_div_up(pair_len4, 256 * 2));
  }
  RB_LAUNCH(k_store_adam_args, dim3(1), dim3(64), stream, a, reinterpret_cast<ClipAdamArgs*>(args_dev));
  RB_LAUNCH_CHECK();
  return rb_launch_adam_pending(reinterpret_cast<const ClipAdamArgs*>(args_dev), (int)grid, stream, target != nullptr);
}

int rb_debug_adam_pass(int32_t form, float* p, float* g, float* m, float* v, int64_t n, const float* part, int32_t nparts,
                       float max_norm, float* norm_out, const long long* step_dev, int64_t step, double lr, double beta1,
                       double beta2, double eps, const int32_t* batch_status, int64_t pair_mu4, int64_t pair_len4, int32_t pair_f4,
                       int32_t pair_split_row, const float* pair_eout, const float* pair_ein, int32_t* pair_clipped, void* args_dev,
                       rb_stream_t stream_) {
  return debug_adam_pass_impl(form, p, g, m, v, n, part, nparts, max_norm, norm_out, step_dev, step, lr, beta1, beta2, eps, batch_status,
                              pair_mu4, pair_len4, pair_f4, pair_split_row, pair_eout, pair_ein, pair_clipped, args_dev, nullptr, 0.0f, stream_);
}
int rb_debug_adam_pass_ema(int32_t form, float* p, float* g, float* m, float* v, int64_t n, const float* part, int32_t nparts,
                           float max_norm, float* norm_out, const long long* step_dev, int64_t step, double lr, double beta1,
                           double beta2, double eps, const int32_t* batch_status, int64_t pair_mu4, int64_t pair_len4, int32_t pair_f4,
                           int32_t pair_split_row, const float* pair_eout, const float* pair_ein, int32_t* pair_clipped, void* args_dev,
                           float* target, float tau, rb_stream_t stream_) {
  RB_REQUIRE(target != nullptr && tau > 0.0f && tau <= 1.0f, "rb_debug_adam_pass_ema: needs a target and tau in (0, 1]");
  return debug_adam_pass_impl(form, p, g, m, v, n, part, nparts, max_norm, norm_out, step_dev, step, lr, beta1, beta2, eps, batch_status,
                              pair_mu4, pair_len4, pair_f4, pair_split_row, pair_eout, pair_ein, pair_clipped, args_dev, target, tau, stream_);
}

int rb_learner_clip_adam_deferred(rb_learner_t* l, float max_norm, float* exp_avg, float* exp_avg_sq, double lr, double beta1,
                                  double beta2, double eps, int64_t step, float* norm_dev, rb_stream_t stream) {
  RB_REQUIRE(l != nullptr, "rb_learner_clip_adam_deferred: NULL handle");
  const int rc = flush_update(l, (hipStream_t)stream);
  if (rc != RB_OK) return rc;
  return clip_adam_impl(l, max_norm, exp_avg, exp_avg_sq, lr, beta1, beta2, eps, step, norm_dev, (hipStream_t)stream,
                        (l->flags & RB_LEARNER_DEFER_UPDATE) != 0);
}

int rb_learner_clip_grad(rb_learner_t* l, float max_norm, float* norm_dev, rb_stream_t stream) {
  RB_REQUIRE(l != nullptr, "rb_learner_clip_grad: NULL handle");
  RB_FLUSH_UPDATE(l, stream);
  RB_MATERIALIZE_SIGMA(l, stream);
  if (l->dw_deferred) {
    rb_set_error("rb_learner_clip_grad: the last learn call left the hidden layer's weight gradient to the fused optimiser "
                 "pass (RB_LEARNER_FUSE_FC_H_DW); call rb_learner_clip_adam, or clear the flag before learning");
    return RB_ERR_STATE;
  }
  const int64_t n = l->L.n_params;
  int nblocks = plan_sumsq_blocks(n);
  int nparts = l->norm_slots;
  if (nparts > 0) {
    if (nblocks > 256) nblocks = 256;
  } else {
    const int rcs = sumsq_pass(l, (hipStream_t)stream, &nparts);
    if (rcs != RB_OK) return rcs;
  }
  l->norm_slots = 0;
  RB_LAUNCH(k_clip_scale, dim3((unsigned)nblocks), dim3(256), stream, l->grads, n, (const float*)l->norm_part, nparts,
            max_norm, norm_dev);
  RB_LAUNCH_CHECK();
  return RB_OK;
}

int rb_learner_clip_adam(rb_learner_t* l, float max_norm, float* exp_avg, float* exp_avg_sq, double lr, double beta1,
                         double beta2, double eps, int64_t step, float* norm_dev, rb_stream_t stream) {
  RB_REQUIRE(l != nullptr, "rb_learner_clip_adam: NULL handle");
  const int rc = flush_update(l, (hipStream_t)stream);
  if (rc != RB_OK) return rc;
  return clip_adam_impl(l, max_norm, exp_avg, exp_avg_sq, lr, beta1, beta2, eps, step, norm_dev, (hipStream_t)stream, false);
}

}
```

Baseline: 6542 gradient-steps/s.

## Split deferred Adam pair update into tenant blocks co-running with conv forward

Splits the deferred Adam update of the noisy-linear paired weights into a hosted head portion plus tail slices. The slices run as extra workgroups appended to the conv2/conv3 forward T16 kernels, which fill CUs that the LDS-limited conv grid leaves idle, and a rest launch covers the remainder before the FC forward. The hosted pass writes a small record (status, clip coef, step size, bc2) so tenant blocks can apply the same update without redoing the norm reduction. This adds planning state, extra argument copies and ordering constraints between the optimizer and the next forward pass.

Result: slower. 6456 gradient-steps/s (-1.3%).

```diff
diff --git a/rainbow_amd/csrc/adam_body.h b/rainbow_amd/csrc/adam_body.h
--- a/rainbow_amd/csrc/adam_body.h
+++ b/rainbow_amd/csrc/adam_body.h
@@ -20,6 +20,8 @@
   const float* pair_ein;
   int32_t* pair_clipped;
   float* t;
+  unsigned pair_lo4, pair_hi4;
+  float* tenant_rec;
 };
 static_assert(sizeof(ClipAdamArgs) <= 256, "ClipAdamArgs: the device copy (adam_args_dev, rb_debug_adam_pass) is 256 bytes");
 __device__ __forceinline__ void rb_adam_elem(float& p, float& g, float& m, float& v, float coef, const ClipAdamArgs& a) {
@@ -91,6 +93,7 @@
   acc = rb_block_sum(acc, s_red16);
   if (rb_wave_uniform(__builtin_bit_cast(int, q.status)) != 0) {
     if (eb == 0 && threadIdx.x == 0 && a.norm_out) rb_st1_wt(a.norm_out, 0, 0.0f);
+    if (eb == 0 && threadIdx.x == 0 && a.tenant_rec) rb_st1_wt(a.tenant_rec, 0, q.status);
     return false;
   }
   const float total = sqrtf(acc);
@@ -99,6 +102,11 @@
   if (eb == 0 && threadIdx.x == 0 && a.norm_out) rb_st1_wt(a.norm_out, 0, total);
   a.neg_step_size = s_red16[16];
   a.bc2_sqrt = s_red16[17];
+  if (eb == 0 && threadIdx.x == 0 && a.tenant_rec) {
+    rb_st1_wt(a.tenant_rec, 0, 0.0f); rb_st1_wt(a.tenant_rec, 4, coef);
+    rb_st1_wt(a.tenant_rec, 8, a.neg_step_size); rb_st1_wt(a.tenant_rec, 12, a.bc2_sqrt);
+    if (a.pair_clipped) rb_st1_wt(reinterpret_cast<float*>(a.pair_clipped), 0, __builtin_bit_cast(float, coef < 1.0f ? 1 : 0));
+  }
   *coef_out = coef;
   return true;
 }
@@ -108,7 +116,8 @@
   constexpr int PU = 2;
   const unsigned T = blockDim.x;
   const unsigned len4 = (unsigned)a.pair_len4, mu4 = (unsigned)a.pair_mu4;
-  const unsigned base = (unsigned)pb * (T * PU) + threadIdx.x;
+  const unsigned lim = a.pair_hi4;
+  const unsigned base = a.pair_lo4 + (unsigned)pb * (T * PU) + threadIdx.x;
   rb_adam_req q;
   rb_adam_hosted_request(a, q);
   const rb_buf beo = rb_make_buf(a.pair_eout), bei = rb_make_buf(a.pair_ein);
@@ -117,7 +126,7 @@
 #pragma unroll
   for (int u = 0; u < PU; ++u) {
     unsigned j = base + u * T;
-    if (j >= len4) j = len4 - 1;
+    if (j >= lim) j = lim - 1;
     const unsigned row = j / (unsigned)a.pair_f4, cq = j - row * (unsigned)a.pair_f4;
     eo[u] = rb_ld1_buf(beo, 4 * row, 0);
     E[u] = rb_ld4_buf(bei, 16 * (cq + ((int)row >= a.pair_split_row ? (unsigned)a.pair_f4 : 0u)), 0);
@@ -127,7 +136,7 @@
 #pragma unroll
   for (int u = 0; u < PU; ++u) {
     unsigned j = base + u * T;
-    if (j >= len4) j = len4 - 1;
+    if (j >= lim) j = lim - 1;
     const unsigned i = mu4 + j, i2 = i + len4;
     P[u] = rb_ld4_buf(bp, 16 * i, 0); G[u] = rb_ld4_buf(bg, 16 * i, 0);
     M[u] = rb_ld4_buf(bm, 16 * i, 0); V[u] = rb_ld4_buf(bv, 16 * i, 0);
@@ -140,17 +149,17 @@
 #pragma unroll
     for (int u = 0; u < PU; ++u) {
       unsigned j = base + u * T;
-      if (j >= len4) j = len4 - 1;
+      if (j >= lim) j = lim - 1;
       TG[u] = rb_ld4_buf(bt, 16 * (mu4 + j), 0); TG2[u] = rb_ld4_buf(bt, 16 * (mu4 + j + len4), 0);
     }
   }
   float coef;
   if (!rb_adam_hosted_prologue(a, eb, q, s_red16, &coef)) return;
-  if (pb == 0 && threadIdx.x == 0 && a.pair_clipped) rb_st1_wt(reinterpret_cast<float*>(a.pair_clipped), 0, __builtin_bit_cast(float, coef < 1.0f ? 1 : 0));
+  if (pb == 0 && threadIdx.x == 0 && a.pair_clipped && !a.tenant_rec) rb_st1_wt(reinterpret_cast<float*>(a.pair_clipped), 0, __builtin_bit_cast(float, coef < 1.0f ? 1 : 0));
 #pragma unroll
   for (int u = 0; u < PU; ++u) {
     const unsigned j = base + u * T;
-    if (j >= len4) continue;
+    if (j >= lim) continue;
     const unsigned i = mu4 + j, i2 = i + len4;
     float4 pr;
     pr.x = eo[u] * E[u].x; pr.y = eo[u] * E[u].y; pr.z = eo[u] * E[u].z; pr.w = eo[u] * E[u].w;
@@ -168,6 +177,58 @@
   }
 }
 
+struct rb_adam_tenant_rec { unsigned status; float coef, neg_step_size, bc2_sqrt; };
+template <bool EMA>
+__device__ __forceinline__ void rb_adam_tenant_pairs(ClipAdamArgs& a, unsigned quad_lo, unsigned quad_hi, const float* rec) {
+  if (quad_lo >= quad_hi) return;
+  const rb_adam_tenant_rec r = rb_ld_uniform(reinterpret_cast<const rb_adam_tenant_rec*>(rec));
+  if (r.status != 0) return;
+  const float coef = r.coef;
+  a.neg_step_size = r.neg_step_size; a.bc2_sqrt = r.bc2_sqrt;
+  const unsigned T = blockDim.x;
+  const unsigned len4 = (unsigned)a.pair_len4, mu4 = (unsigned)a.pair_mu4, f4 = (unsigned)a.pair_f4;
+  const rb_buf beo = rb_make_buf(a.pair_eout), bei = rb_make_buf(a.pair_ein);
+  const rb_buf bp = rb_make_buf(a.p), bg = rb_make_buf(a.g), bm = rb_make_buf(a.m), bv = rb_make_buf(a.v);
+  const bool ema_copy = EMA && a.tau == 1.0f;
+  const rb_buf bt = rb_make_buf(EMA ? a.t : a.p);
+  struct Trip { float4 P, G, M, V, P2, M2, V2, E, TG, TG2; float eo; };
+  auto request = [&](unsigned j, Trip& t) {
+    if (j >= quad_hi) j = quad_hi - 1;
+    const unsigned row = j / f4, cq = j - row * f4;
+    const unsigned i = mu4 + j, i2 = i + len4;
+    t.eo = rb_ld1_buf(beo, 4 * row, 0);
+    t.E = rb_ld4_buf(bei, 16 * (cq + ((int)row >= a.pair_split_row ? f4 : 0u)), 0);
+    t.P = rb_ld4_buf(bp, 16 * i, 0); t.G = rb_ld4_buf(bg, 16 * i, 0);
+    t.M = rb_ld4_buf(bm, 16 * i, 0); t.V = rb_ld4_buf(bv, 16 * i, 0);
+    t.P2 = rb_ld4_buf(bp, 16 * i2, 0); t.M2 = rb_ld4_buf(bm, 16 * i2, 0); t.V2 = rb_ld4_buf(bv, 16 * i2, 0);
+    if (EMA && !ema_copy) { t.TG = rb_ld4_buf(bt, 16 * i, 0); t.TG2 = rb_ld4_buf(bt, 16 * i2, 0); }
+  };
+  Trip cur, nxt;
+  request(quad_lo + threadIdx.x, cur);
+  for (unsigned j0 = quad_lo; j0 < quad_hi; j0 += T) {
+    const bool more = j0 + T < quad_hi;
+    if (more) request(j0 + T + threadIdx.x, nxt);
+    const unsigned j = j0 + threadIdx.x;
+    if (j < quad_hi) {
+      const unsigned i = mu4 + j, i2 = i + len4;
+      float4 pr;
+      pr.x = cur.eo * cur.E.x; pr.y = cur.eo * cur.E.y; pr.z = cur.eo * cur.E.z; pr.w = cur.eo * cur.E.w;
+      float4 G2;
+      G2.x = cur.G.x * pr.x; G2.y = cur.G.y * pr.y; G2.z = cur.G.z * pr.z; G2.w = cur.G.w * pr.w;
+      rb_adam_quad(cur.P, cur.G, cur.M, cur.V, coef, a);
+      rb_adam_quad(cur.P2, G2, cur.M2, cur.V2, coef, a);
+      rb_st4_wt(a.p, 16 * i, cur.P); rb_st4_wt(a.m, 16 * i, cur.M); rb_st4_wt(a.v, 16 * i, cur.V);
+      rb_st4_wt(a.p, 16 * i2, cur.P2); rb_st4_wt(a.m, 16 * i2, cur.M2); rb_st4_wt(a.v, 16 * i2, cur.V2);
+      if (coef < 1.0f) { rb_st4_wt(a.g, 16 * i, cur.G); rb_st4_wt(a.g, 16 * i2, G2); }
+      if (EMA) {
+        rb_ema_quad(cur.TG, cur.P, a.tau, ema_copy); rb_ema_quad(cur.TG2, cur.P2, a.tau, ema_copy);
+        rb_st4_wt(a.t, 16 * i, cur.TG); rb_st4_wt(a.t, 16 * i2, cur.TG2);
+      }
+    }
+    if (more) cur = nxt;
+  }
+}
+
 template <int UNROLL, bool EMA = false>
 __device__ __forceinline__ void rb_adam_hosted_block(const ClipAdamArgs* ad, int eb, int nblk, float* s_red16 ) {
   ClipAdamArgs a = rb_ld_uniform(ad);
diff --git a/rainbow_amd/csrc/conv_dispatch.h b/rainbow_amd/csrc/conv_dispatch.h
--- a/rainbow_amd/csrc/conv_dispatch.h
+++ b/rainbow_amd/csrc/conv_dispatch.h
@@ -40,6 +40,17 @@
   a.rows_total = n_on + n_tg;
   a.ipb = p.ipb;
   a.img_fast = p.img_fast;
+  a.tn_ad = nullptr; a.tn_lo = a.tn_hi = 0; a.tn_x0 = 0; a.tn_n = 0; a.tn_ema = 0;
+  dim3 grid = p.grid;
+  if (l->adam_rest && p.kernel == CONV_FWD_T16 && p.img_fast && !FIRST) {
+    const AdamTenantPlan& tn = l->adam_tn;
+    const int i = l->adam_rest - 1;
+    if (i < tn.n && tn.layer[i] == layer) {
+      a.tn_ad = adam_args_block(l, 1); a.tn_lo = tn.lo[i]; a.tn_hi = tn.lo[i + 1];
+      a.tn_x0 = (int)p.grid.x; a.tn_n = tn.wgs[i]; a.tn_ema = l->adam_args_host.t != nullptr ? 1 : 0;
+      grid.x += (unsigned)tn.extra_x[i];
+    }
+  }
   static const char* const tags[3] = {"conv1_fwd:k_conv_fwd_lds", "conv2_fwd:k_conv_fwd_lds", "conv3_fwd:k_conv_fwd_lds"};
   const dim3 block(p.block);
   switch (p.kernel) {
@@ -50,7 +61,7 @@
       if constexpr (!FIRST && C::T16_OK) { RB_LAUNCH_T(tags[layer], (k_conv_fwd_multi_t16<G, NT, PR, KMAX, PCH>), p.grid, block, stream, a); }
       break;
     case CONV_FWD_T16:
-      if constexpr (C::T16_OK) { RB_LAUNCH_T(tags[layer], (k_conv_fwd_t16<G, NT, PR, KMAX, FIRST, PCH, 1>), p.grid, block, stream, a); }
+      if constexpr (C::T16_OK) { RB_LAUNCH_T(tags[layer], (k_conv_fwd_t16<G, NT, PR, KMAX, FIRST, PCH, 1>), grid, block, stream, a); }
       break;
     case CONV_FWD_LDS_F32:
       if constexpr (FIRST) { RB_LAUNCH_T(tags[layer], (k_conv_fwd_lds<G, NT, PR, KMAX, FIRST, PCH, FIRST>), p.grid, block, stream, a); }
@@ -61,6 +72,7 @@
     case CONV_FWD_GEMM: break;
   }
   RB_LAUNCH_CHECK();
+  if (a.tn_ad) l->adam_rest = l->adam_rest < l->adam_tn.n ? l->adam_rest + 1 : 0;
   return RB_OK;
 }
 
diff --git a/rainbow_amd/csrc/conv_fwd.h b/rainbow_amd/csrc/conv_fwd.h
--- a/rainbow_amd/csrc/conv_fwd.h
+++ b/rainbow_amd/csrc/conv_fwd.h
@@ -1,6 +1,7 @@
 #pragma once
 #include "conv_stage.h"
 #include "kernel_stamp.h"
+#include "adam_body.h"
 
 struct ConvLdsFwdArgs {
   int cin, cout;
@@ -14,7 +15,22 @@
   int rows_total;
   int ipb;
   int img_fast;
+  const ClipAdamArgs* tn_ad;
+  unsigned tn_lo, tn_hi;
+  int tn_x0, tn_n, tn_ema;
 };
+
+__device__ __forceinline__ void rb_conv_fwd_tenant(const ConvLdsFwdArgs& a) {
+  const unsigned ex = gridDim.x - (unsigned)a.tn_x0;
+  const unsigned t = (blockIdx.x - (unsigned)a.tn_x0) + ex * (blockIdx.y + gridDim.y * blockIdx.z);
+  if (t >= (unsigned)a.tn_n) return;
+  const unsigned chunk = ((a.tn_hi - a.tn_lo + (unsigned)a.tn_n - 1) / (unsigned)a.tn_n + 15u) & ~15u;
+  const unsigned lo = a.tn_lo + t * chunk;
+  const unsigned hi = lo + chunk < a.tn_hi ? lo + chunk : a.tn_hi;
+  ClipAdamArgs ad = rb_ld_uniform(a.tn_ad);
+  if (a.tn_ema) rb_adam_tenant_pairs<true>(ad, lo, hi, ad.tenant_rec);
+  else rb_adam_tenant_pairs<false>(ad, lo, hi, ad.tenant_rec);
+}
 
 template <class G>
 __device__ __forceinline__ void rb_conv_store_out(const ConvLdsFwdArgs& a, int img, int m, int p, float o) {
@@ -525,6 +541,9 @@
 template <class G, int NT, int PR, int KMAX, bool FIRST, int PCH = 32 * NT, int CTW = 1>
 __global__ __launch_bounds__((64 * ConvFwdWaves<G, NT, PR, KMAX, FIRST, PCH, false, CTW>::NWV))
 void k_conv_fwd_t16(ConvLdsFwdArgs a) {
+  if constexpr (!FIRST) {
+    if (a.tn_ad != nullptr && (int)blockIdx.x >= a.tn_x0) { rb_conv_fwd_tenant(a); return; }
+  }
   __shared__ __attribute__((aligned(16))) float smem[ConvFwdLdsSize<G, NT, PR, KMAX, CTW>::FLOATS + ConvFwdWaves<G, NT, PR, KMAX, FIRST, PCH, false, CTW>::PARTF];
   if (a.img_fast) rb_conv_fwd_body<G, NT, PR, KMAX, FIRST, PCH, false, CTW>(a, (int)blockIdx.z, (int)blockIdx.y, (int)blockIdx.x, smem);
   else rb_conv_fwd_body<G, NT, PR, KMAX, FIRST, PCH, false, CTW>(a, (int)blockIdx.x, (int)blockIdx.y, (int)blockIdx.z, smem);
diff --git a/rainbow_amd/csrc/fc_dispatch.h b/rainbow_amd/csrc/fc_dispatch.h
--- a/rainbow_amd/csrc/fc_dispatch.h
+++ b/rainbow_amd/csrc/fc_dispatch.h
@@ -83,10 +83,12 @@
 
 static int forward(rb_learner* l, int n_on, int n_tg, const ImgSrc& src, const NetPtrs& on, const NetPtrs& tg,
                    hipStream_t stream) {
+  if (l->adam_rest && !(n_on == 2 * l->L.B && n_tg == l->L.B && src.f32 == nullptr && l->caps.fast_conv)) RB_FLUSH_UPDATE_REST(l, stream);
   for (int layer = 0; layer < l->L.nconv; ++layer) {
     int rc = conv_fwd(l, layer, n_on, n_tg, src, on, tg, stream);
     if (rc != RB_OK) return rc;
   }
+  RB_FLUSH_UPDATE_REST(l, stream);
   return fc_forward(l, n_on, n_tg, on, tg, stream);
 }
 
diff --git a/rainbow_amd/csrc/launch_plan_debug.h b/rainbow_amd/csrc/launch_plan_debug.h
--- a/rainbow_amd/csrc/launch_plan_debug.h
+++ b/rainbow_amd/csrc/launch_plan_debug.h
@@ -18,15 +18,27 @@
   }
 };
 
-static void plan_text_forward(PlanText& t, const PlanIn& in, const char* prefix, int n_on, int n_tg, bool f32) {
+static void plan_text_forward(PlanText& t, const PlanIn& in, const char* prefix, int n_on, int n_tg, bool f32, int64_t tenant_pair_len4 = -1) {
   const Layout& L = in.L;
+  ConvFwdPlan fwd[3];
+  for (int layer = 0; layer < L.nconv; ++layer) fwd[layer] = plan_conv_fwd(in, layer, n_on, n_tg, f32);
+  const AdamTenantPlan tn = plan_adam_tenants(in, fwd, tenant_pair_len4 > 0, tenant_pair_len4);
   for (int layer = 0; layer < L.nconv; ++layer) {
-    const ConvFwdPlan p = plan_conv_fwd(in, layer, n_on, n_tg, f32);
+    const ConvFwdPlan p = fwd[layer];
     char name[96];
     if (p.kernel == CONV_FWD_GEMM) snprintf(name, sizeof(name), "k_gemm<ConvFwdProb<%s>>", p.geom);
     else snprintf(name, sizeof(name), "%s<%s%s>", conv_fwd_kernel_name[p.kernel], p.geom, p.kernel == CONV_FWD_LDS_F32 ? ",F32SRC" : "");
-    t.line("%sconv%d_fwd kernel=%s grid=%ux%ux%u block=%u ipb=%d img_fast=%d", prefix, layer + 1, name, p.grid.x, p.grid.y, p.grid.z,
-           p.block, p.ipb, p.img_fast);
+    if (tenant_pair_len4 < 0) {
+      t.line("%sconv%d_fwd kernel=%s grid=%ux%ux%u block=%u ipb=%d img_fast=%d", prefix, layer + 1, name, p.grid.x, p.grid.y, p.grid.z,
+             p.block, p.ipb, p.img_fast);
+      continue;
+    }
+    int i = -1;
+    for (int k = 0; k < tn.n; ++k)
+      if (tn.layer[k] == layer) i = k;
+    t.line("%sconv%d_fwd kernel=%s grid=%ux%ux%u block=%u ipb=%d img_fast=%d adam_tenants=%d adam_quads=%u/%u adam_pair_quads=%lld", prefix,
+           layer + 1, name, p.grid.x, p.grid.y, p.grid.z, p.block, p.ipb, p.img_fast, i >= 0 ? tn.wgs[i] : 0, i >= 0 ? tn.lo[i] : 0u,
+           i >= 0 ? tn.lo[i + 1] : 0u, (long long)tenant_pair_len4);
   }
   const FcFwdPlan f = plan_fc_fwd(in, n_on, n_tg);
   if (f.block_copy) t.line("%sfeat_block_copy kernel=k_block_copy", prefix);
@@ -52,7 +64,10 @@
   out[0] = 0;
   t.line("caps fast_fc=%d fast_conv=%d hs=%d xs=%d ws=%d/%d/%d wT=%d/%d/%d gemm_ws=%d", caps.fast_fc, caps.fast_conv, caps.hs, caps.xs,
          caps.ws[0], caps.ws[1], caps.ws[2], caps.wT[0], caps.wT[1], caps.wT[2], caps.gemm_ws);
-  plan_text_forward(t, in, "", 2 * L.B, L.B, false);
+  {
+    const bool pairing = (flags & RB_LEARNER_DEFER_UPDATE) != 0 && plan_fc_bwd(in, false).implicit_sigma;
+    plan_text_forward(t, in, "", 2 * L.B, L.B, false, pairing ? (int64_t)2 * L.H * L.F / 4 : 0);
+  }
   {
     const HeadPlan h = plan_head(in);
     t.line("head kernel=k_head<%d> grid=%ux1x1 block=%d samples=%d tenants=%d waves=%d wt_t16=%d/%d", h.ZI, h.blocks, 64 * h.waves, L.B,
diff --git a/rainbow_amd/csrc/learner.hip b/rainbow_amd/csrc/learner.hip
--- a/rainbow_amd/csrc/learner.hip
+++ b/rainbow_amd/csrc/learner.hip
@@ -49,7 +49,7 @@
   float** owned[] = {&l->feat_b, &l->h_b, &l->act[0], &l->act[1], &l->act[2], &l->dact[0], &l->dact[1], &l->dact[2], &l->hpart, &l->h,
                      &l->logits, &l->dlogits, &l->dlogitsT, &l->dh, &l->dhT, &l->dfeat_part, &l->dw_part[0], &l->dw_part[1], &l->dw_part[2],
                      &l->conv_wT[0], &l->conv_wT[1], &l->conv_wT[2],
-                     &l->log_ps_a, &l->pns_a, &l->m, &l->support, &l->zero_noise, &l->norm_part, &l->gemm_part, &l->noise_snap, &l->feat_s, &l->h_s};
+                     &l->log_ps_a, &l->pns_a, &l->m, &l->support, &l->zero_noise, &l->norm_part, &l->gemm_part, &l->noise_snap, &l->feat_s, &l->h_s, &l->adam_rec};
   for (float** p : owned)
     if (*p) rb_dev_free(*p);
   if (l->a_star) rb_dev_free(l->a_star);
@@ -205,7 +205,8 @@
   RB_ALLOC(l->norm_part, RB_NORM_PART_SLOTS);
   RB_ALLOC(l->noise_ctr, 4);
   RB_ALLOC(l->status_copy, 4);
-  RB_ALLOC(l->adam_args_dev, (sizeof(ClipAdamArgs) + 3) / 4);
+  RB_ALLOC(l->adam_args_dev, 4 * 256 / 4);
+  RB_ALLOC(l->adam_rec, 4);
   RB_ALLOC(l->act_ctr, 6 * RB_FAN_SHARDS * RB_FAN_STRIDE + 32);
 #undef RB_ALLOC
   RB_HIP_TRY(hipMemset(l->act_ctr, 0, (6 * RB_FAN_SHARDS * RB_FAN_STRIDE + 32) * 4));
@@ -331,7 +332,7 @@
                              const float* weights_dev, float* loss_dev, rb_stream_t stream_) {
   RB_REQUIRE(l && frames_dev && windows_dev && actions_dev && returns_dev && nonterminals_dev && weights_dev && loss_dev,
              "rb_learner_learn_windows: NULL argument");
-  RB_FLUSH_UPDATE(l, stream_);
+  if (!l->adam_rest) RB_FLUSH_UPDATE(l, stream_);
   RB_REQUIRE(window_len == l->L.hist + l->cfg.multi_step, "rb_learner_learn_windows: window_len must be history + multi_step");
   if (!l->caps.fast_conv) {
     rb_set_error("rb_learner_learn_windows: zero-copy frames need the LDS conv kernels (history <= 4); gather the stacks and "
@@ -349,8 +350,11 @@
   rb_noise_job_t hosted_job;
   const rb_noise_job_t* job = a->noise_job;
   bool hosted = false;
+  RB_FLUSH_UPDATE_REST(l, stream);
+  const bool split = l->adam_pending && l->adam_tn.n > 0 && comm == nullptr && !l->opt.spec_draw && a->window_len <= 24 &&
+                     a->window_len == l->L.hist + l->cfg.multi_step && l->caps.fast_conv;
   if (l->adam_pending) {
-    if (job != nullptr && attach_pending_pass(l, job, a->batch, &hosted_job)) {
+    if (job != nullptr && attach_pending_pass(l, job, a->batch, &hosted_job, split)) {
       job = &hosted_job;
       hosted = true;
     } else {
@@ -381,10 +385,17 @@
                                         nullptr, a->actions_dev, a->returns_dev, a->nonterminals_dev, a->weights_dev,
                                         job, stream);
   if (rc != RB_OK) { l->spec_now = 0; return rc; }
-  if (hosted) l->adam_pending = 0;
+  if (hosted) {
+    l->adam_pending = 0;
+    if (split) l->adam_rest = 1;
+  }
   rc = rb_learner_learn_windows(l, a->frames_dev, rb_replay_current_windows(a->replay), a->window_len, a->actions_dev, a->returns_dev,
                                 a->nonterminals_dev, a->weights_dev, a->loss_dev, stream);
   l->spec_now = 0;
+  if (l->adam_rest) {
+    const int rcr = flush_rest(l, (hipStream_t)stream);
+    if (rc == RB_OK) rc = rcr;
+  }
   {
     auto& t = l->ts_last;
     t.replay = a->replay; t.batch = a->batch; t.max_attempts = a->max_attempts; t.beta = a->priority_weight; t.tree_idx = a->tree_idx_dev;
diff --git a/rainbow_amd/csrc/learner_internal.h b/rainbow_amd/csrc/learner_internal.h
--- a/rainbow_amd/csrc/learner_internal.h
+++ b/rainbow_amd/csrc/learner_internal.h
@@ -109,7 +109,7 @@
 }
 
 struct RbOpts {
-  int generic, fc_gemm, implicit_small, xs, act_fused, spec_draw, spec_stall, img_fast, conv_multi, conv_full, t16, dx_ipb, dw_ipb0, dw_ipb1, dw_ipb2;
+  int generic, fc_gemm, implicit_small, xs, act_fused, spec_draw, spec_stall, img_fast, conv_multi, conv_full, t16, dx_ipb, dw_ipb0, dw_ipb1, dw_ipb2, adam_tenants;
 };
 static const struct { const char* key; int RbOpts::*field; int dflt; const char* what; } rb_opt_table[] = {
   {"generic", &RbOpts::generic, 0, "1: every contraction on the gemm_core.h fallback; 2: the noisy-linear layers only"},
@@ -127,6 +127,8 @@
   {"dw_ipb0", &RbOpts::dw_ipb0, 0, "images per workgroup of conv layer 0 in the weight-gradient launch: 0 = by shape"},
   {"dw_ipb1", &RbOpts::dw_ipb1, 0, "... of conv layer 1"},
   {"dw_ipb2", &RbOpts::dw_ipb2, 0, "... of conv layer 2"},
+  {"adam_tenants", &RbOpts::adam_tenants, 0, "megabytes of the pending optimiser pass's pair range per forward launch of conv layers 2 and 3, run by "
+   "tenant workgroups on the CUs those launches leave free (0: none); test hook: -((workgroups << 20) | quads) per launch"},
 };
 static int rb_opts_parse(const char* s, RbOpts* o) {
   for (const auto& row : rb_opt_table) o->*row.field = row.dflt;
@@ -155,6 +157,13 @@
   int hs, xs, ws[3];
   int wT[3];
   int gemm_ws;
+};
+
+struct AdamTenantPlan {
+  int n;
+  int layer[2];
+  int wgs[2], extra_x[2];
+  unsigned lo[3];
 };
 
 struct rb_learner {
@@ -217,6 +226,10 @@
   ClipAdamArgs* adam_args_dev;
   ClipAdamArgs adam_args_host;
   int adam_args_valid, adam_pending, adam_blocks;
+  AdamTenantPlan adam_tn;
+  int adam_host_blocks;
+  int adam_rest;
+  float* adam_rec;
   float target_tau;
   unsigned* go_flag;
   unsigned go_epoch;
@@ -231,7 +244,12 @@
   float delta_z;
 };
 
+static ClipAdamArgs* adam_args_block(rb_learner* l, int i) {
+  return reinterpret_cast<ClipAdamArgs*>(reinterpret_cast<char*>(l->adam_args_dev) + 256 * i);
+}
+
 static int flush_update(rb_learner* l, hipStream_t stream);
+static int flush_rest(rb_learner* l, hipStream_t stream);
 static int materialize_sigma(rb_learner* l, hipStream_t stream);
 int rb_comm_world(const rb_comm_t* comm);
 int rb_comm_all_gather_f32(rb_comm_t* comm, const float* send, float* recv, size_t count, hipStream_t stream);
@@ -239,6 +257,11 @@
 #define RB_FLUSH_UPDATE(l, stream)                                  \
   do {                                                              \
     const int rcf_ = flush_update((l), (hipStream_t)(stream));      \
+    if (rcf_ != RB_OK) return rcf_;                                 \
+  } while (0)
+#define RB_FLUSH_UPDATE_REST(l, stream)                             \
+  do {                                                              \
+    const int rcf_ = flush_rest((l), (hipStream_t)(stream));        \
     if (rcf_ != RB_OK) return rcf_;                                 \
   } while (0)
 #define RB_MATERIALIZE_SIGMA(l, stream)                             \
diff --git a/rainbow_amd/csrc/learner_plan.h b/rainbow_amd/csrc/learner_plan.h
--- a/rainbow_amd/csrc/learner_plan.h
+++ b/rainbow_amd/csrc/learner_plan.h
@@ -84,6 +84,7 @@
   dim3 grid;
   unsigned block;
   int ipb, img_fast;
+  int lds_bytes;
   const char* geom;
 };
 template <class C>
@@ -92,7 +93,7 @@
   const ConvLayer& c = in.L.conv[layer];
   const int NI = n_on + n_tg;
   ConvFwdPlan p;
-  p.ipb = 1; p.img_fast = 0; p.geom = C::name;
+  p.ipb = 1; p.img_fast = 0; p.lds_bytes = 0; p.geom = C::name;
   if (!in.caps.fast_conv) {
     const int n_max = (n_on > n_tg ? n_on : n_tg) * G::P;
     p.kernel = CONV_FWD_GEMM; p.grid = dim3(1, (unsigned)rb_div_up(n_max, layer == 0 ? 64 : 32), 2); p.block = 128;
@@ -135,6 +136,7 @@
   if constexpr (C::T16_OK) {
     if (!C::FIRST || (in.opt.t16 && !f32 && c.cin * G::KK == C::KMAX)) {
       p.kernel = CONV_FWD_T16; p.block = 64 * ConvFwdWaves<G, C::NT, C::PR, C::KMAX, C::FIRST, C::PCH, false, 1>::NWV;
+      p.lds_bytes = 4 * (int)(ConvFwdLdsSize<G, C::NT, C::PR, C::KMAX, 1>::FLOATS + ConvFwdWaves<G, C::NT, C::PR, C::KMAX, C::FIRST, C::PCH, false, 1>::PARTF);
       return p;
     }
   }
@@ -143,6 +145,40 @@
 }
 static ConvFwdPlan plan_conv_fwd(const PlanIn& in, int layer, int n_on, int n_tg, bool f32) {
   return with_geom(in.L.conv[layer], [&](auto cfg) { return plan_conv_fwd_g<decltype(cfg)>(in, layer, n_on, n_tg, f32); });
+}
+
+#define RB_LDS_BYTES_PER_CU (160 * 1024)
+#define RB_ADAM_PAIR_QUAD_BYTES 208
+static AdamTenantPlan plan_adam_tenants(const PlanIn& in, const ConvFwdPlan* fwd, bool hosted, int64_t pair_len4) {
+  AdamTenantPlan t;
+  memset(&t, 0, sizeof(t));
+  const int v = in.opt.adam_tenants;
+  if (!hosted || pair_len4 <= 0 || v == 0 || in.exch) return t;
+  const int forced_wgs = v < 0 ? (int)((unsigned)(-v) >> 20) : 0;
+  const int64_t per_launch = v < 0 ? (int64_t)((unsigned)(-v) & 0xfffffu) : (int64_t)v * 1000000 / RB_ADAM_PAIR_QUAD_BYTES;
+  unsigned q[2] = {0, 0};
+  int64_t left = pair_len4;
+  for (int layer = 1; layer < in.L.nconv && t.n < 2; ++layer) {
+    const ConvFwdPlan& p = fwd[layer];
+    if (p.kernel != CONV_FWD_T16 || p.ipb != 1 || !p.img_fast) continue;
+    if (2 * p.lds_bytes <= RB_LDS_BYTES_PER_CU) continue;
+    const int real = (int)(p.grid.x * p.grid.y * p.grid.z), per_x = (int)(p.grid.y * p.grid.z);
+    int wgs = forced_wgs > 0 ? forced_wgs : in.n_cu - real;
+    if (wgs <= 0) continue;
+    int ex = (int)rb_div_up(wgs, per_x);
+    if (forced_wgs > 0) ex = (int)rb_div_up(ex, 8) * 8;
+    else { ex = wgs / per_x / 8 * 8; wgs = ex * per_x; }
+    if (ex <= 0) continue;
+    const int64_t take = per_launch < left ? per_launch : left;
+    t.layer[t.n] = layer; t.wgs[t.n] = wgs; t.extra_x[t.n] = ex; q[t.n] = (unsigned)take;
+    left -= take;
+    ++t.n;
+  }
+  t.lo[0] = (unsigned)left;
+  t.lo[1] = t.lo[0] + q[0];
+  t.lo[2] = t.lo[1] + q[1];
+  if (t.n == 1) t.lo[2] = t.lo[1];
+  return t;
 }
 
 static constexpr bool dx_t16_geom(int ks, int s, int ih) { return (ks == 4 && s == 2 && ih == 20) || (ks == 3 && s == 1 && ih == 9); }
diff --git a/rainbow_amd/csrc/optimizer_host.h b/rainbow_amd/csrc/optimizer_host.h
--- a/rainbow_amd/csrc/optimizer_host.h
+++ b/rainbow_amd/csrc/optimizer_host.h
@@ -13,7 +13,20 @@
   return RB_OK;
 }
 
+static int flush_rest(rb_learner* l, hipStream_t stream) {
+  if (!l->adam_rest) return RB_OK;
+  const int64_t quads = l->adam_args_host.pair_len4 - (int64_t)l->adam_tn.lo[l->adam_rest - 1];
+  const int which = 1 + l->adam_rest;
+  l->adam_rest = 0;
+  if (quads <= 0) return RB_OK;
+  return rb_launch_adam_pending(adam_args_block(l, which), (int)rb_div_up(quads, 256 * 2), stream, l->adam_args_host.t != nullptr);
+}
+
 static int flush_update(rb_learner* l, hipStream_t stream) {
+  {
+    const int rcr = flush_rest(l, stream);
+    if (rcr != RB_OK) return rcr;
+  }
   if (!l->adam_pending) return RB_OK;
   FusedDwAdamArgs f;
   memset(&f, 0, sizeof(f));
@@ -40,11 +53,11 @@
   return RB_OK;
 }
 
-static bool attach_pending_pass(rb_learner* l, const rb_noise_job_t* job_in, int32_t batch, rb_noise_job_t* job_out) {
+static bool attach_pending_pass(rb_learner* l, const rb_noise_job_t* job_in, int32_t batch, rb_noise_job_t* job_out, bool split = false) {
   memcpy(job_out, job_in, sizeof(*job_out));
   if (!l->adam_pending || batch > 256) return false;
   NoiseJob* nj = reinterpret_cast<NoiseJob*>(job_out);
-  nj->adam_dev = l->adam_args_dev; nj->adam_blocks = l->adam_blocks;
+  nj->adam_dev = split ? adam_args_block(l, 1) : l->adam_args_dev; nj->adam_blocks = split ? l->adam_host_blocks : l->adam_blocks;
   nj->adam_ema = l->adam_args_host.t != nullptr ? 1 : 0;
   return true;
 }
@@ -113,6 +126,7 @@
       a.pair_mu4 = L.h_mu / 4; a.pair_len4 = (int64_t)2 * L.H * L.F / 4;
       a.pair_f4 = L.F / 4; a.pair_split_row = L.H; a.pair_eout = sn.h_eout; a.pair_ein = sn.h_ein;
       a.pair_clipped = l->status_copy + 2;
+      a.pair_lo4 = 0; a.pair_hi4 = (unsigned)a.pair_len4;
       a.hole_lo4 = (unsigned)a.pair_mu4; a.hole4 = (unsigned)(2 * a.pair_len4);
       a.pair_blk0 = (int)rb_div_up(n4 - 2 * a.pair_len4 > 0 ? n4 - 2 * a.pair_len4 : 1, 256 * 4);
       grid = (unsigned)(a.pair_blk0 + rb_div_up(a.pair_len4, 256 * 2));
@@ -121,14 +135,35 @@
       if (rcm != RB_OK) return rcm;
     }
     if (will_defer) {
-      if (!l->adam_args_valid || memcmp(&a, &l->adam_args_host, sizeof(a)) != 0) {
+      AdamTenantPlan tn;
+      {
+        const PlanIn in = plan_in(l);
+        ConvFwdPlan fwd[3];
+        for (int layer = 0; layer < l->L.nconv; ++layer) fwd[layer] = plan_conv_fwd(in, layer, 2 * l->L.B, l->L.B, false);
+        tn = plan_adam_tenants(in, fwd, true, a.pair_len4);
+      }
+      if (!l->adam_args_valid || memcmp(&a, &l->adam_args_host, sizeof(a)) != 0 || memcmp(&tn, &l->adam_tn, sizeof(tn)) != 0) {
         RB_LAUNCH(k_store_adam_args, dim3(1), dim3(64), stream, a, l->adam_args_dev);
         RB_LAUNCH_CHECK();
+        if (tn.n > 0) {
+          ClipAdamArgs s1 = a;
+          s1.pair_hi4 = tn.lo[0]; s1.tenant_rec = l->adam_rec;
+          RB_LAUNCH(k_store_adam_args, dim3(1), dim3(64), stream, s1, adam_args_block(l, 1));
+          RB_LAUNCH_CHECK();
+          for (int r = 0; r < 2; ++r) {
+            ClipAdamArgs s2 = a;
+            s2.pair_blk0 = 0; s2.pair_lo4 = tn.lo[r]; s2.norm_out = nullptr; s2.pair_clipped = nullptr;
+            RB_LAUNCH(k_store_adam_args, dim3(1), dim3(64), stream, s2, adam_args_block(l, 2 + r));
+            RB_LAUNCH_CHECK();
+          }
+        }
         memcpy(&l->adam_args_host, &a, sizeof(a));
+        memcpy(&l->adam_tn, &tn, sizeof(tn));
         l->adam_args_valid = 1;
       }
       l->adam_pending = 1;
       l->adam_blocks = (int)grid;
+      l->adam_host_blocks = a.pair_blk0 + (int)rb_div_up((int64_t)tn.lo[0], 256 * 2);
       return RB_OK;
     }
     if (ema) RB_LAUNCH_T("clip_adam:k_clip_adam", (k_clip_adam<4, true, false, true>), dim3(grid), dim3(256), stream, a, f);
@@ -206,6 +241,7 @@
                "rb_debug_adam_pass: bad pair range");
     a.pair_mu4 = pair_mu4; a.pair_len4 = pair_len4; a.pair_f4 = pair_f4; a.pair_split_row = pair_split_row;
     a.pair_eout = pair_eout; a.pair_ein = pair_ein; a.pair_clipped = pair_clipped;
+    a.pair_lo4 = 0; a.pair_hi4 = (unsigned)pair_len4;
     a.hole_lo4 = (unsigned)pair_mu4; a.hole4 = (unsigned)(2 * pair_len4);
     a.pair_blk0 = (int)rb_div_up(n4 - 2 * pair_len4 > 0 ? n4 - 2 * pair_len4 : 1, 256 * 4);
     grid = (unsigned)(a.pair_blk0 + rb_div_up(pair_len4, 256 * 2));
```
